# ZikangXiong/mobrob

Measured on AMD Instinct MI355X. Metric: env-steps/sec (whole node), doggo PPO, higher is better.
Workload: dtype f32

## Files before the change

### mobrob_amd/csrc/engine.hip

```cpp
#include <hip/hip_runtime.h>
#include <rccl/rccl.h>
#include <dlfcn.h>

#include <algorithm>
#include <atomic>
#include <thread>
#include <cmath>
#include <cstdarg>
#include <cstdio>
#include <climits>
#include <cstring>
#include <ctime>
#include <cstdlib>
#include <string>
#include <vector>

#ifdef MOBROB_POISON_LDS
namespace mobrob {
__global__ __launch_bounds__(1024) void k_poison_lds() {
  extern __shared__ unsigned poison_words[];
  volatile unsigned* w = poison_words;
  for (int i = threadIdx.x; i < 160 * 256; i += 1024) w[i] = 0xFFFFFFFFu;
}
inline void poison_lds(hipStream_t st) {
// ... 88 lines not shown
  int HL = 0, GL = 0;
  int tPW[kMaxHidden] = {0}, tPB[kMaxHidden] = {0}, tVW[kMaxHidden] = {0}, tVB[kMaxHidden] = {0}, tAW = 0, tAB = 0, tVWh = 0, tVBh = 0;
  int ntens = 13;
  int Bl;
  int nmb;
  int rows_max;
  int offs[kMaxTensors + 1];
  hipStream_t stream = nullptr;
  bool own_stream = false;
  float *params = nullptr, *grads = nullptr , *m = nullptr, *v = nullptr;
  NormChunk* chunks_dev = nullptr;
  double* chunk_partial = nullptr;
  int nchunks = 0;
  float *pW1p = nullptr, *vW1p = nullptr, *aWp = nullptr, *vWp = nullptr;
  int64_t adam_step = 0;
  float *obs = nullptr, *actions = nullptr, *rewards = nullptr, *es = nullptr, *values = nullptr, *logp = nullptr,
        *adv = nullptr, *ret = nullptr;
  float *last_values = nullptr, *last_dones = nullptr, *prev_dones = nullptr, *dones_tmp = nullptr;
  float *clip_act = nullptr, *rew_tmp = nullptr, *term_obs = nullptr, *term_val = nullptr, *eps_dev = nullptr;
  uint8_t *trunc_dev = nullptr, *dones_u8 = nullptr;
  int *ep_len = nullptr, *ep_len2 = nullptr;
  uint32_t* ctr_dev = nullptr;
  hipGraph_t ro_graph = nullptr;
  hipGraphExec_t ro_exec = nullptr;
  struct RolloutSpec {
    int kind = 0;
    float p_term = 0.f;
    int time_limit = 0;
    GoalEnvParams goal{};
  } ro_spec;
  int env_started = 0;
  hipStream_t vstream = nullptr;
  std::vector<hipEvent_t> ev_chunks;
  hipEvent_t ev_vdone = nullptr;
  float* gstate[2] = {nullptr, nullptr};
  double* ep_stats = nullptr;
  uint64_t ep_ring_read = 0;
  uint32_t draw_counter = 0;
  int nparts = 0;
  int part_act_t[MOBROB_MAX_PARTS] = {0}, part_store_t[MOBROB_MAX_PARTS] = {0};
  int part_obs_t[MOBROB_MAX_PARTS] = {0};
  hipEvent_t ev_part[MOBROB_MAX_PARTS] = {nullptr};
  const void* pinned_seen[8] = {nullptr};
  unsigned pinned_seen_n = 0;
  uint32_t draw_ro0 = 0;
  unsigned* srv_flags = nullptr;
  int srv_blocks = 0;
  int* srv_abort = nullptr;
  uint32_t env_step_counter = 0;
  int t = 0;
  bool rollout_ready = false;
  bool train_rec_valid = false;
  bool train_rec_external = false;
  int* rows = nullptr;
  int64_t* perm_dev = nullptr;
  double* advstat = nullptr;
  double* expvar_part = nullptr;
  unsigned long long* advbins = nullptr;
  uint64_t perm_counter = 0;
  unsigned adv_pass = 0;
  bool epoch_open = false;
  float* stats = nullptr;
  int stats_cap = 0, stats_n = 0;
  int cur_count = 0;
  bool grad_pending = false;
  double clip_vf = -1.0;
  double target_kl = -1.0;
  int last_epochs_started = 0, last_stopped_early = 0, last_steps_applied = 0;
  ncclComm_t comm = nullptr;
  int64_t allreduce_calls = 0, allreduce_bytes = 0;
  struct OneShot {
    char* xbuf = nullptr;
    size_t payload = 0;
    char* peer[kOneShotMaxRanks] = {nullptr};
    int world = 0, rank = -1;
    bool ready = false;
    unsigned long long seq = 0;
    int* error = nullptr;
    long long timeout_ticks = 0;
  } oneshot;
  double* norm_rec_sum = nullptr; int* norm_rec_t = nullptr; int* fold_idx_dev = nullptr;
  int fold_start[kMaxTensors + 1] = {0};
  bool use_norm_records = false;
  bool epoch_kernel_on = true;
  unsigned* epoch_bar = nullptr;
  float* epoch_consts = nullptr;
  int* epoch_idx = nullptr;
  char* epoch_stage = nullptr;
  int* epoch_err_host = nullptr;
  hipEvent_t epoch_ev = nullptr;
  int last_update_mode = 0;
  float* epoch_snap = nullptr;
  int rollout64_tile_max = 256;
  int pair64_min_tiles = 65;
  int split64_max_tiles = 64;
  float *Xg = nullptr, *actg = nullptr, *lpg = nullptr, *advg = nullptr, *retg = nullptr, *oldvg = nullptr;
  float *hp[kMaxHidden] = {nullptr}, *hv[kMaxHidden] = {nullptr}, *mu = nullptr, *vout = nullptr;
  float *dmu = nullptr, *dv = nullptr, *dzp[kMaxHidden] = {nullptr}, *dzv[kMaxHidden] = {nullptr};
  float *pred_obs = nullptr, *pred_act = nullptr;
  int gemm_tiles = 0;
  bool sde = false, sde_hold = false;
  float *sde_E = nullptr, *sde_E1 = nullptr, *sde_lat2 = nullptr, *sde_gsig = nullptr, *sde_graw = nullptr;
  float *sde_S2 = nullptr, *sde_var = nullptr;
  SdeMode sde_mode{1, 0};
  hipStream_t cstream = nullptr;
  hipEvent_t ev_in = nullptr, ev_k = nullptr, ev_store = nullptr;
  struct Stage {
    float *obs = nullptr, *eps = nullptr, *rew = nullptr, *term = nullptr;
    uint8_t *dones = nullptr, *trunc = nullptr;
  } stage[2];
  float *o_raw = nullptr, *o_clip = nullptr, *o_val = nullptr, *o_lp = nullptr;
  int stage_i = 0;
  bool prof_on = false;
  uint32_t prof_mask = ~0u;
  std::vector<ProfSpan> spans;
  std::vector<hipEvent_t> ev_pool;
  double prof_ms[MOBROB_K_COUNT] = {0};
  int64_t prof_calls[MOBROB_K_COUNT] = {0};
  std::vector<void*> allocs;
  char* arena = nullptr;
  size_t arena_bytes = 0, arena_used = 0;
  bool plan_only = false;
  std::vector<NormChunk> chunk_table;
  FusedState fused;
  char* eval_buf = nullptr;
  size_t eval_bytes = 0;
};

namespace {

int check_async_error(mobrob_ppo_engine* e);

constexpr size_t kArenaAlign = 256;

template <typename Tp>
int dalloc(mobrob_ppo_engine* e, Tp** p, size_t count) {
  const size_t bytes = (std::max<size_t>(count, 1) * sizeof(Tp) + kArenaAlign - 1) / kArenaAlign * kArenaAlign;
  if (e->plan_only) {
    e->arena_used += bytes;
    *p = nullptr;
    return MOBROB_OK;
  }
  if (e->arena_used + bytes > e->arena_bytes)
    return fail(MOBROB_ERR_INVALID, "device arena too small: need more than %zu bytes", e->arena_bytes);
  void* q = e->arena + e->arena_used;
  e->arena_used += bytes;
  HIPC(hipMemsetAsync(q, 0, bytes, e->stream));
  *p = static_cast<Tp*>(q);
  return MOBROB_OK;
}

hipEvent_t get_event(mobrob_ppo_engine* e) {
  if (!e->ev_pool.empty()) {
    hipEvent_t ev = e->ev_pool.back();
    e->ev_pool.pop_back();
    return ev;
  }
  hipEvent_t ev;
  (void)hipEventCreate(&ev);
  return ev;
}

struct ProfScope {
  mobrob_ppo_engine* e;
  ProfSpan s;
  bool on;
// ... 69 lines not shown
}
int gemm_tile_class(const mobrob_ppo_engine* e, const GemmOp& a) {
  const int f = e->gemm_tiles, M = a.g.M, N = a.g.N;
  if (f == 22 && M > 32 && N > 32) return 22;
  if ((f == 21 || f == 22) && M > 32) return 21;
  const long w21 = (long)cdiv(M, 64) * cdiv(N, 32) * a.ksplit, w22 = (long)cdiv(M, 64) * cdiv(N, 64) * a.ksplit;
  if (f != 0 || M <= 32 || w21 < 2048) return 11;
  return (N <= 32 || w22 < 2048) ? 21 : 22;
}
void launch_multi(mobrob_ppo_engine* e, const GemmOp* const* ops, int n) {
  GemmMulti m{};
  int gx = 1, gy = 1, z = 0;
  for (int p = 0; p < 4; ++p) {
    const GemmOp& o = *ops[p < n ? p : n - 1];
    m.g[p] = o.g; m.mode[p] = o.mode; m.epi[p] = o.epi;
    m.zbeg[p] = z;
    if (p < n) {
      z += o.ksplit;
      gx = std::max(gx, cdiv(cdiv(o.g.M, 32), 4)); gy = std::max(gy, cdiv(o.g.N, 32));
    }
  }
  m.zbeg[4] = z;
  hipLaunchKernelGGL(k_gemm_multi, dim3(gx, gy, z), dim3(256), 0, e->stream, m);
}
void run_queues(mobrob_ppo_engine* e, const GemmQueue& qa, const GemmQueue& qb, int width) {
  static const int pairing = env_int("MOBROB_GEMM_PAIR", 2);
  const size_t n = std::max(qa.size(), qb.size());
  for (size_t j0 = 0; j0 < n; j0 += width) {
    const GemmOp* st[4];
    int ns = 0;
    bool small = pairing >= 2;
    for (size_t j = j0; j < j0 + width && j < n; ++j)
      for (const GemmQueue* q : {&qa, &qb})
        if (j < q->size()) {
          st[ns++] = &(*q)[j];
          small = small && gemm_tile_class(e, (*q)[j]) == 11;
        }
    if (small && ns >= 2) { launch_multi(e, st, ns); continue; }
    for (size_t j = j0; j < j0 + width && j < n; ++j) {
      const GemmOp* a = j < qa.size() ? &qa[j] : nullptr;
      const GemmOp* b = j < qb.size() ? &qb[j] : nullptr;
      if (a && b && pairing >= 1 && a->mode == b->mode && a->epi == b->epi) { launch_op(e, *a, b); continue; }
      if (a) launch_op(e, *a);
      if (b) launch_op(e, *b);
    }
  }
}

void linear_fwd(mobrob_ppo_engine* e, const float* X, int ldx, const float* W, int ldw, const float* bias, float* Y,
                int ldy, int M, int Nn, int K, bool tanh_, float* Z = nullptr, GemmQueue* q = nullptr) {
  GemmOp o;
  GemmArgs& g = o.g;
  g.A = X; g.B = W; g.C = Y; g.M = M; g.N = Nn; g.K = K; g.lda = ldx; g.ldb = ldw; g.ldc = ldy; g.bias = bias;
  g.act = e->cfg.activation;
  g.Z = (tanh_ && act_needs_z(g.act)) ? Z : nullptr; g.ldz = ldy;
  o.mode = MODE_NT; o.epi = tanh_ ? EPI_BIAS_TANH : EPI_BIAS;
  if (q) q->push_back(o); else launch_op(e, o);
}
void linear_bwd_input(mobrob_ppo_engine* e, const float* dY, int ldd, const float* W, int ldw, const float* H, int ldh,
                      float* dZ, int ldz, float* bias_grad, int M, int Nn, int K, GemmQueue* q = nullptr) {
  GemmOp o;
  GemmArgs& g = o.g;
  g.A = dY; g.B = W; g.C = dZ; g.M = M; g.N = Nn; g.K = K; g.lda = ldd; g.ldb = ldw; g.ldc = ldz;
  g.Hact = H; g.ldh = ldh; g.colsum = bias_grad; g.act = e->cfg.activation;
  o.mode = MODE_NN; o.epi = EPI_DTANH_COLSUM;
  if (q) q->push_back(o); else launch_op(e, o);
}
void linear_bwd_weight(mobrob_ppo_engine* e, const float* dY, int ldd, const float* X, int ldx, float* dW, int ldw,
                       int M, int Nn, int rows, GemmQueue* q = nullptr) {
  GemmOp o;
  GemmArgs& g = o.g;
  g.A = dY; g.B = X; g.C = dW; g.M = M; g.N = Nn; g.K = rows; g.lda = ldd; g.ldb = ldx; g.ldc = ldw;
  const int wtiles = cdiv(M, M <= 32 ? 32 : 64) * cdiv(Nn, (M <= 32 || Nn <= 32) ? 32 : 64);
  int ksplit = std::max(1, std::min(cdiv(rows, 64), cdiv(2048, wtiles)));
  g.kchunk = rup(cdiv(rows, ksplit), 8);
  o.ksplit = cdiv(rows, g.kchunk);
  o.mode = MODE_TN; o.epi = EPI_ATOMIC;
  if (q) q->push_back(o); else launch_op(e, o);
}

float* Pp(mobrob_ppo_engine* e, int t) { return e->params + e->offs[t]; }
float* Gp(mobrob_ppo_engine* e, int t) { return e->grads + e->offs[t]; }

void pack_x3_all(mobrob_ppo_engine* e) {
  if (e->fused.net[0].W2x == nullptr) return;
  PackX3Args a{};
  const int w1[2] = {T_PW1, T_VW1}, w2[2] = {T_PW2, T_VW2};
  int maxthreads = 0;
  for (int n = 0; n < 2; ++n) {
    const int i1 = 3 * n, i2 = 3 * n + 1, i3 = 3 * n + 2;
    a.W[i1] = Pp(e, w1[n]); a.N[i1] = FH; a.K[i1] = e->D; a.ld[i1] = e->D; a.NB[i1] = FH / 32; a.KS[i1] = e->Dp / 16; a.scale[i1] = kTanhScale;
    a.out[i1] = reinterpret_cast<unsigned short*>(const_cast<unsigned*>(e->fused.net[n].W1x));
    a.W[i2] = Pp(e, w2[n]); a.N[i2] = FH; a.K[i2] = FH; a.ld[i2] = FH; a.NB[i2] = FH / 32; a.KS[i2] = FH / 16; a.scale[i2] = kTanhScale;
    a.out[i2] = reinterpret_cast<unsigned short*>(const_cast<unsigned*>(e->fused.net[n].W2x));
    a.W[i3] = Pp(e, w2[n]); a.N[i3] = FH; a.K[i3] = FH; a.ld[i3] = FH; a.NB[i3] = FH / 32; a.KS[i3] = FH / 16; a.scale[i3] = 1.0f; a.trans[i3] = 1;
    a.out[i3] = reinterpret_cast<unsigned short*>(const_cast<unsigned*>(e->fused.net[n].W2bx));
    maxthreads = std::max(maxthreads, std::max(a.NB[i1] * a.KS[i1], a.NB[i2] * a.KS[i2]) * 512);
  }
  hipLaunchKernelGGL(k_pack_x3_multi, dim3(cdiv(maxthreads, 256), 6), dim3(256), 0, e->stream, a);
  if (e->fused.train_chain) {
    ChainPackArgs c{};
    const int w3[2] = {T_AW, T_VW};
    for (int n = 0; n < 2; ++n) {
      c.W1[n] = Pp(e, w1[n]); c.W2[n] = Pp(e, w2[n]); c.W3[n] = Pp(e, w3[n]);
      c.w1c[n] = reinterpret_cast<unsigned short*>(const_cast<unsigned*>(e->fused.net[n].W1c));
      c.w2c[n] = reinterpret_cast<unsigned short*>(const_cast<unsigned*>(e->fused.net[n].W2c));
      c.w2bc[n] = reinterpret_cast<unsigned short*>(const_cast<unsigned*>(e->fused.net[n].W2bc));
      c.w3c[n] = const_cast<float*>(e->fused.net[n].W3c); c.w3bc[n] = const_cast<float*>(e->fused.net[n].W3bc);
      c.head[n] = n == 0 ? e->A : 1;
    }
    c.D = e->D; c.Dp = e->Dp;
    hipLaunchKernelGGL(k_pack_chain, dim3(FH * FH / 256, 2), dim3(256), 0, e->stream, c);
  }
}

void repack(mobrob_ppo_engine* e) {
  auto pad = [&](const float* src, float* dst, int r, int c, int rp, int cp) {
    hipLaunchKernelGGL(k_pad_rows, dim3(cdiv(rp * cp, 256)), dim3(256), 0, e->stream, src, dst, r, c, rp, cp);
  };
  pad(Pp(e, T_PW1), e->pW1p, e->H1, e->D, e->H1, e->Dp);
  pad(Pp(e, T_VW1), e->vW1p, e->G1, e->D, e->G1, e->Dp);
  pad(Pp(e, T_AW), e->aWp, e->A, e->HL, e->Ap, e->HL);
  pad(Pp(e, T_VW), e->vWp, 1, e->GL, 8, e->GL);
  fused_repack(e->fused, e->params, e->offs, e->stream);
  pack_x3_all(e);
}

void forward_generic(mobrob_ppo_engine* e, const float* X, int rows, bool want_pi, float* mu_out, bool want_v,
                     float* v_out, bool keep_z = false) {
  GemmQueue qp, qv;
  if (want_pi) {
    linear_fwd(e, X, e->Dp, e->pW1p, e->Dp, Pp(e, e->tPB[0]), e->hp[0], e->Hp[0], rows, e->Hp[0], e->Dp, true, keep_z ? e->dzp[0] : nullptr, &qp);
    for (int l = 1; l < e->Lp; ++l)
      linear_fwd(e, e->hp[l - 1], e->Hp[l - 1], Pp(e, e->tPW[l]), e->Hp[l - 1], Pp(e, e->tPB[l]), e->hp[l], e->Hp[l], rows, e->Hp[l], e->Hp[l - 1], true,
                 keep_z ? e->dzp[l] : nullptr, &qp);
    linear_fwd(e, e->hp[e->Lp - 1], e->HL, e->aWp, e->HL, Pp(e, T_AB), mu_out, e->Ap, rows, e->A, e->HL, false, nullptr, &qp);
  }
  if (want_v) {
    linear_fwd(e, X, e->Dp, e->vW1p, e->Dp, Pp(e, e->tVB[0]), e->hv[0], e->Hv[0], rows, e->Hv[0], e->Dp, true, keep_z ? e->dzv[0] : nullptr, &qv);
    for (int l = 1; l < e->Lv; ++l)
      linear_fwd(e, e->hv[l - 1], e->Hv[l - 1], Pp(e, e->tVW[l]), e->Hv[l - 1], Pp(e, e->tVB[l]), e->hv[l], e->Hv[l], rows, e->Hv[l], e->Hv[l - 1], true,
                 keep_z ? e->dzv[l] : nullptr, &qv);
    linear_fwd(e, e->hv[e->Lv - 1], e->GL, e->vWp, e->GL, Pp(e, T_VB), v_out, 1, rows, 1, e->GL, false, nullptr, &qv);
  }
  run_queues(e, qp, qv, 1);
}

void forward(mobrob_ppo_engine* e, const float* X, int rows, bool want_pi, float* mu_out, bool want_v, float* v_out) {
  if (e->fused.enabled && fused_forward(e->fused, X, rows, want_pi, mu_out, e->Ap, want_v, v_out, e->stream)) return;
  forward_generic(e, X, rows, want_pi, mu_out, want_v, v_out);
}

int value_net_width_sum(const mobrob_ppo_engine* e) {
  int s = 0;
  for (int l = 0; l < e->Lv; ++l) s += e->Hv[l];
  return s;
}
ValueNetArgs value_net_args(mobrob_ppo_engine* e) {
  ValueNetArgs vn{};
  for (int l = 0; l < e->Lv; ++l) { vn.W[l] = Pp(e, e->tVW[l]); vn.b[l] = Pp(e, e->tVB[l]); vn.G[l] = e->Hv[l]; }
  vn.Wv = Pp(e, T_VW); vn.bv = Pp(e, T_VB);
  vn.L = e->Lv; vn.act = e->cfg.activation; vn.width_sum = value_net_width_sum(e);
  return vn;
}
BootNetArgs boot_args(mobrob_ppo_engine* e) { return BootNetArgs{value_net_args(e), (float)e->cfg.gamma, e->term_val}; }

void value_flagged(mobrob_ppo_engine* e, const float* obs_rows, const uint8_t* flags, float* out,
                   float* bootstrap_rewards = nullptr) {
  const size_t sm = (size_t)(e->D + value_net_width_sum(e) + 16) * sizeof(float);
  hipLaunchKernelGGL(k_value_flagged, dim3(e->N), dim3(256), sm, e->stream, obs_rows, e->Dp, flags, value_net_args(e), e->D, out,
                     bootstrap_rewards, (float)e->cfg.gamma);
}

uint64_t eps_seed(const mobrob_ppo_engine* e) { return e->cfg.seed ^ (0xD1B54A32D192ED03ull * (uint64_t)(e->cfg.rank + 1)); }

void run_gae(mobrob_ppo_engine* e) {
  ProfScope ps(e, MOBROB_K_GAE);
  const double gl = e->cfg.gamma * e->cfg.gae_lambda;
  hipLaunchKernelGGL(k_gae, dim3(cdiv(e->N, kGaeEnvs)), dim3(kGaeThreads), 0, e->stream, e->rewards, e->values, e->es, e->last_values,
                     e->last_dones, (float)e->cfg.gamma, gl, e->T, e->N, e->adv, e->ret);
}

void sde_resample(mobrob_ppo_engine* e, int r0, int n, uint32_t draw, const uint32_t* draw_base, bool single) {
  const int HLA = e->HL * e->A, per = cdiv(HLA, 4);
  hipLaunchKernelGGL(k_sde_resample, dim3(cdiv((n + (single ? 1 : 0)) * per, 256)), dim3(256), 0, e->stream, Pp(e, T_LOGSTD), HLA, e->A, e->sde_mode, r0, n,
                     eps_seed(e) ^ 0x5DE5DE5DE5DE5DEull, draw, draw_base, e->sde_E, single ? e->sde_E1 : (float*)nullptr);
}

void sde_variance(mobrob_ppo_engine* e, int rows, bool fresh_table, float* lat2 = nullptr) {
  if (fresh_table)
    hipLaunchKernelGGL(k_sde_std2, dim3(cdiv(e->HL * e->A, 256)), dim3(256), 0, e->stream, Pp(e, T_LOGSTD), e->HL, e->A, e->sde_mode, e->sde_S2);
  hipLaunchKernelGGL(k_sde_var, dim3(cdiv(rows, 4)), dim3(256), 0, e->stream, e->hp[e->Lp - 1], e->HL, e->sde_S2, rows, e->HL, e->A, e->sde_var, e->Ap,
                     lat2);
}

void act_rows(mobrob_ppo_engine* e, int t, int r0, int n, const float* eps_dev_or_null, uint32_t draw,
              const uint32_t* draw_base, float* clip_out = nullptr) {
  ProfScope ps(e, MOBROB_K_ACT);
  if (!clip_out) clip_out = e->clip_act + (size_t)r0 * e->A;
  const size_t row = (size_t)t * e->N + r0;
  const float* X = e->obs + row * e->Dp;
  if (e->fused.enabled) {
    FusedActArgs a{};
    a.X = X; a.rows = n; a.row0 = r0; a.want_pi = 1; a.want_v = 1; a.mu = nullptr; a.ldmu = e->Ap;
    a.v = e->values + row; a.sample = 1; a.A = e->A; a.log_std = Pp(e, T_LOGSTD); a.eps = eps_dev_or_null;
    a.seed = eps_seed(e); a.draw = draw; a.draw_base = draw_base; a.lo = (float)e->cfg.action_low; a.hi = (float)e->cfg.action_high;
    a.act_raw = e->actions + row * e->A; a.act_clip = clip_out; a.logp = e->logp + row;
    fused_launch_act(e->fused, a, e->stream);
// ... 648 lines not shown
    }
    (void)hipHostFree(e->o_raw); (void)hipHostFree(e->o_clip); (void)hipHostFree(e->o_val); (void)hipHostFree(e->o_lp);
    (void)hipEventDestroy(e->ev_in); (void)hipEventDestroy(e->ev_k); (void)hipEventDestroy(e->ev_store);
    (void)hipStreamDestroy(e->cstream);
  }
  for (hipEvent_t ev : e->ev_part)
    if (ev) (void)hipEventDestroy(ev);
  if (e->srv_flags) (void)hipHostFree(e->srv_flags);
  if (e->srv_abort) (void)hipFree(e->srv_abort);
  if (e->epoch_stage) (void)hipHostFree(e->epoch_stage);
  if (e->epoch_err_host) (void)hipHostFree(e->epoch_err_host);
  if (e->epoch_ev) (void)hipEventDestroy(e->epoch_ev);
  if (e->ro_exec) (void)hipGraphExecDestroy(e->ro_exec);
  if (e->ro_graph) (void)hipGraphDestroy(e->ro_graph);
  if (e->vstream) {
    (void)hipStreamSynchronize(e->vstream);
    for (auto ev : e->ev_chunks) (void)hipEventDestroy(ev);
    (void)hipEventDestroy(e->ev_vdone);
    (void)hipStreamDestroy(e->vstream);
  }
  for (auto ev : e->ev_pool) (void)hipEventDestroy(ev);
  for (void* p : e->allocs) (void)hipFree(p);
  if (e->eval_buf) (void)hipFree(e->eval_buf);
  if (e->own_stream && e->stream) (void)hipStreamDestroy(e->stream);
  delete e;
}

int mobrob_ppo_set_stream(mobrob_ppo_engine_t* e, void* s) {
  if (!e) return fail(MOBROB_ERR_INVALID, "null engine");
  HIPC(hipStreamSynchronize(e->stream));
  if (e->ro_exec) { (void)hipGraphExecDestroy(e->ro_exec); e->ro_exec = nullptr; }
  if (e->ro_graph) { (void)hipGraphDestroy(e->ro_graph); e->ro_graph = nullptr; }
  if (e->own_stream && e->stream) HIPC(hipStreamDestroy(e->stream));
  if (s == nullptr) {
    HIPC(hipStreamCreateWithFlags(&e->stream, hipStreamNonBlocking));
    e->own_stream = true;
  } else {
    e->stream = static_cast<hipStream_t>(s);
    e->own_stream = false;
  }
  return MOBROB_OK;
}

int mobrob_ppo_synchronize(mobrob_ppo_engine_t* e) {
  if (!e) return fail(MOBROB_ERR_INVALID, "null engine");
  HIPC(hipStreamSynchronize(e->stream));
  return check_async_error(e);
}

int64_t mobrob_ppo_param_count(const mobrob_ppo_engine_t* e) { return e ? e->P : -1; }

int mobrob_ppo_get_params(mobrob_ppo_engine_t* e, float* out, int64_t n) {
  if (!e || !out || n != e->P) return fail(MOBROB_ERR_INVALID, "get_params: n=%lld, expected %d", (long long)n, e ? e->P : -1);
  HIPC(hipMemcpyAsync(out, e->params, (size_t)n * 4, hipMemcpyDeviceToHost, e->stream));
  HIPC(hipStreamSynchronize(e->stream));
  return MOBROB_OK;
}
int mobrob_ppo_set_params(mobrob_ppo_engine_t* e, const float* in, int64_t n) {
  if (!e || !in || n != e->P) return fail(MOBROB_ERR_INVALID, "set_params: n=%lld, expected %d", (long long)n, e ? e->P : -1);
  HIPC(hipMemcpyAsync(e->params, in, (size_t)n * 4, hipMemcpyHostToDevice, e->stream));
  repack(e);
  HIPC(hipStreamSynchronize(e->stream));
  return MOBROB_OK;
}
int mobrob_ppo_get_optimizer_state(mobrob_ppo_engine_t* e, float* m, float* v, int64_t n, int64_t* step) {
  if (!e || n != e->P) return fail(MOBROB_ERR_INVALID, "get_optimizer_state: bad size");
  if (m) HIPC(hipMemcpyAsync(m, e->m, (size_t)n * 4, hipMemcpyDeviceToHost, e->stream));
  if (v) HIPC(hipMemcpyAsync(v, e->v, (size_t)n * 4, hipMemcpyDeviceToHost, e->stream));
  HIPC(hipStreamSynchronize(e->stream));
  if (step) *step = e->adam_step;
  return MOBROB_OK;
}
int mobrob_ppo_set_optimizer_state(mobrob_ppo_engine_t* e, const float* m, const float* v, int64_t n, int64_t step) {
  if (!e || !m || !v || n != e->P || step < 0) return fail(MOBROB_ERR_INVALID, "set_optimizer_state: bad argument");
  HIPC(hipMemcpyAsync(e->m, m, (size_t)n * 4, hipMemcpyHostToDevice, e->stream));
  HIPC(hipMemcpyAsync(e->v, v, (size_t)n * 4, hipMemcpyHostToDevice, e->stream));
  HIPC(hipStreamSynchronize(e->stream));
  e->adam_step = step;
  return MOBROB_OK;
}

int mobrob_ppo_rollout_begin(mobrob_ppo_engine_t* e) {
  if (!e) return fail(MOBROB_ERR_INVALID, "null engine");
  e->t = 0;
  e->rollout_ready = false; e->train_rec_valid = false;
  e->nparts = 0;
  for (auto& q : e->pinned_seen) q = nullptr;
  e->pinned_seen_n = 0;
  e->draw_ro0 = e->draw_counter;
  for (int p = 0; p < MOBROB_MAX_PARTS; ++p) {
    e->part_act_t[p] = e->part_store_t[p] = 0;
    e->part_obs_t[p] = -1;
  }
  return MOBROB_OK;
}

int mobrob_ppo_act(mobrob_ppo_engine_t* e, const float* obs, const float* eps, float* a_raw, float* a_clip,
                   float* values, float* logp) {
  if (!e || !obs) return fail(MOBROB_ERR_INVALID, "act: null argument");
  if (e->t >= e->T) return fail(MOBROB_ERR_STATE, "act: rollout buffer full (t=%d, n_steps=%d)", e->t, e->T);
  CHK(streamer_init(e));
  const size_t N = e->N, A = e->A, D = e->D;
  if (!eps && is_pinned(obs) && (!a_raw || is_pinned(a_raw)) && (!a_clip || is_pinned(a_clip)) &&
      (!values || is_pinned(values)) && (!logp || is_pinned(logp))) {
    hipLaunchKernelGGL(k_pull_rows, dim3(cdiv((int)(N * e->Dp), 256)), dim3(256), 0, e->stream, obs,
                       e->obs + (size_t)e->t * N * e->Dp, (int)N, (int)D, e->Dp);
    act_slot(e, e->t, nullptr);
    auto push = [&](const float* dev, float* host, size_t n) {
      if (host) hipLaunchKernelGGL(k_copy_f32, dim3(cdiv((int)n, 256)), dim3(256), 0, e->stream, dev, host, (int)n);
    };
    push(e->clip_act, a_clip, N * A);
    push(e->actions + (size_t)e->t * N * A, a_raw, N * A);
    push(e->values + (size_t)e->t * N, values, N);
    push(e->logp + (size_t)e->t * N, logp, N);
    HIPC(hipGetLastError());
    HIPC(hipStreamSynchronize(e->stream));
    return MOBROB_OK;
  }
  auto& st = e->stage[e->stage_i];
  const float* src = stage_in(obs, st.obs, N * D);
  CHK(upload_obs_on(e, e->cstream, src, e->obs + (size_t)e->t * N * e->Dp, e->N));
  if (eps) {
    const float* es = stage_in(eps, st.eps, N * A);
    HIPC(hipMemcpyAsync(e->eps_dev, es, N * A * 4, hipMemcpyHostToDevice, e->cstream));
  }
  HIPC(hipEventRecord(e->ev_in, e->cstream));
  HIPC(hipStreamWaitEvent(e->stream, e->ev_in, 0));
  act_slot(e, e->t, eps ? e->eps_dev : nullptr);
  HIPC(hipEventRecord(e->ev_k, e->stream));
  HIPC(hipStreamWaitEvent(e->cstream, e->ev_k, 0));
  struct Out { float* user; float* stagebuf; const float* dev; size_t n; };
  const Out outs[4] = {{a_clip, e->o_clip, e->clip_act, N * A},
                       {a_raw, e->o_raw, e->actions + (size_t)e->t * N * A, N * A},
                       {values, e->o_val, e->values + (size_t)e->t * N, N},
                       {logp, e->o_lp, e->logp + (size_t)e->t * N, N}};
  bool staged[4] = {false, false, false, false};
  for (int i = 0; i < 4; ++i) {
    if (!outs[i].user) continue;
    staged[i] = !is_pinned(outs[i].user);
    HIPC(hipMemcpyAsync(staged[i] ? outs[i].stagebuf : outs[i].user, outs[i].dev, outs[i].n * 4, hipMemcpyDeviceToHost,
                        e->cstream));
  }
  HIPC(hipStreamSynchronize(e->cstream));
  for (int i = 0; i < 4; ++i)
    if (outs[i].user && staged[i]) memcpy(outs[i].user, outs[i].stagebuf, outs[i].n * 4);
  return MOBROB_OK;
}

namespace {
bool any_truncated(const uint8_t* truncated, const float* terminal_obs, int r0, int n) {
  bool any = false;
  if (truncated && terminal_obs)
    for (int i = r0; i < r0 + n; ++i) any |= truncated[i] != 0;
  return any;
}
void store_step(mobrob_ppo_engine* e, const float* rew, const uint8_t* dones, bool any_trunc) {
  const size_t o = (size_t)e->t * e->N;
  if (any_trunc) value_flagged(e, e->term_obs, e->trunc_dev, e->term_val);
  hipLaunchKernelGGL(k_store_step, dim3(cdiv(e->N, 256)), dim3(256), 0, e->stream, rew, e->prev_dones,
                     any_trunc ? e->trunc_dev : nullptr, e->term_val, (float)e->cfg.gamma, e->N, e->rewards + o, e->es + o);
  hipLaunchKernelGGL(k_u8_to_f32, dim3(cdiv(e->N, 256)), dim3(256), 0, e->stream, dones, e->prev_dones, e->N);
}
}

int mobrob_ppo_store(mobrob_ppo_engine_t* e, const float* rewards, const uint8_t* dones, const uint8_t* truncated,
                     const float* terminal_obs) {
  if (!e || !rewards || !dones) return fail(MOBROB_ERR_INVALID, "store: null argument");
  if (e->t >= e->T) return fail(MOBROB_ERR_STATE, "store: rollout buffer full");
  CHK(streamer_init(e));
  const size_t N = e->N, D = e->D;
  const bool any_trunc = any_truncated(truncated, terminal_obs, 0, e->N);
  if (is_pinned(rewards) && is_pinned(dones) && (!truncated || is_pinned(truncated)) &&
      (!terminal_obs || is_pinned(terminal_obs))) {
    if (any_trunc) {
      hipLaunchKernelGGL(k_pull_rows, dim3(cdiv((int)(N * e->Dp), 256)), dim3(256), 0, e->stream, terminal_obs, e->term_obs,
                         (int)N, (int)D, e->Dp);
      HIPC(hipMemcpyAsync(e->trunc_dev, truncated, N, hipMemcpyHostToDevice, e->stream));
    }
    store_step(e, rewards, dones, any_trunc);
    HIPC(hipGetLastError());
    e->t++;
    return MOBROB_OK;
  }
  auto& st = e->stage[e->stage_i];
  memcpy(st.rew, rewards, N * 4);
  memcpy(st.dones, dones, N);
  HIPC(hipMemcpyAsync(e->rew_tmp, st.rew, N * 4, hipMemcpyHostToDevice, e->cstream));
  HIPC(hipMemcpyAsync(e->dones_u8, st.dones, N, hipMemcpyHostToDevice, e->cstream));
  if (any_trunc) {
    memcpy(st.trunc, truncated, N);
    memcpy(st.term, terminal_obs, N * D * 4);
    HIPC(hipMemcpyAsync(e->trunc_dev, st.trunc, N, hipMemcpyHostToDevice, e->cstream));
    CHK(upload_obs_on(e, e->cstream, st.term, e->term_obs, e->N));
  }
  HIPC(hipEventRecord(e->ev_store, e->cstream));
  HIPC(hipStreamWaitEvent(e->stream, e->ev_store, 0));
  store_step(e, e->rew_tmp, e->dones_u8, any_trunc);
  HIPC(hipEventRecord(e->ev_k, e->stream));
  HIPC(hipStreamWaitEvent(e->cstream, e->ev_k, 0));
  HIPC(hipGetLastError());
  e->stage_i ^= 1;
  e->t++;
  return MOBROB_OK;
}

namespace {
int part_range(mobrob_ppo_engine* e, int part, int nparts, int* r0, int* n) {
  if (nparts < 1 || nparts > MOBROB_MAX_PARTS || nparts > e->N || part < 0 || part >= nparts)
    return fail(MOBROB_ERR_INVALID, "part %d of %d (1..%d parts, at most one per env)", part, nparts, MOBROB_MAX_PARTS);
  if (e->nparts == 0) e->nparts = nparts;
  if (e->nparts != nparts) return fail(MOBROB_ERR_STATE, "nparts changed from %d to %d inside a rollout", e->nparts, nparts);
  *r0 = (int)((int64_t)e->N * part / nparts);
  *n = (int)((int64_t)e->N * (part + 1) / nparts) - *r0;
  return MOBROB_OK;
}
}

int mobrob_ppo_act_part(mobrob_ppo_engine_t* e, int32_t part, int32_t nparts, const float* obs, float* a_clip) {
  if (!e || !obs || !a_clip) return fail(MOBROB_ERR_INVALID, "act_part: null argument");
  int r0, n;
  CHK(part_range(e, part, nparts, &r0, &n));
  const int t = e->part_act_t[part];
  if (t >= e->T) return fail(MOBROB_ERR_STATE, "act_part: rollout buffer full (part %d, t=%d)", part, t);
  if (t != e->part_store_t[part]) return fail(MOBROB_ERR_STATE, "act_part: part %d acted on step %d but has not stored it", part, t - 1);
  if (!is_pinned_cached(e, obs) || !is_pinned_cached(e, a_clip))
    return fail(MOBROB_ERR_INVALID, "act_part needs device-visible pinned buffers (mobrob_ppo_host_alloc)");
  if (!e->ev_part[part]) HIPC(hipEventCreateWithFlags(&e->ev_part[part], hipEventDisableTiming));
  const size_t D = e->D, A = e->A;
  if (e->part_obs_t[part] != t)
    hipLaunchKernelGGL(k_pull_rows, dim3(cdiv(n * e->Dp, 256)), dim3(256), 0, e->stream, obs + (size_t)r0 * D,
                       e->obs + ((size_t)t * e->N + r0) * e->Dp, n, (int)D, e->Dp);
  act_rows(e, t, r0, n, nullptr, e->draw_ro0 + (uint32_t)t, nullptr, a_clip + (size_t)r0 * A);
  HIPC(hipGetLastError());
  HIPC(hipEventRecord(e->ev_part[part], e->stream));
  e->part_act_t[part] = t + 1;
  if (e->draw_counter < e->draw_ro0 + (uint32_t)t + 1) e->draw_counter = e->draw_ro0 + (uint32_t)t + 1;
  return MOBROB_OK;
}

int mobrob_ppo_wait_part(mobrob_ppo_engine_t* e, int32_t part) {
  if (!e || part < 0 || part >= MOBROB_MAX_PARTS || !e->ev_part[part])
    return fail(MOBROB_ERR_STATE, "wait_part: part %d has no act_part in flight", part);
  HIPC(hipEventSynchronize(e->ev_part[part]));
  return MOBROB_OK;
}

int mobrob_ppo_store_part(mobrob_ppo_engine_t* e, int32_t part, int32_t nparts, const float* rewards,
                          const uint8_t* dones, const uint8_t* truncated, const float* terminal_obs,
                          const float* next_obs) {
  if (!e || !rewards || !dones) return fail(MOBROB_ERR_INVALID, "store_part: null argument");
  int r0, n;
  CHK(part_range(e, part, nparts, &r0, &n));
  const int t = e->part_store_t[part];
  if (t + 1 != e->part_act_t[part]) return fail(MOBROB_ERR_STATE, "store_part: part %d has no acted step to store (t=%d)", part, t);
  if (!is_pinned_cached(e, rewards) || !is_pinned_cached(e, dones) || (truncated && !is_pinned_cached(e, truncated)) ||
      (terminal_obs && !is_pinned_cached(e, terminal_obs)) || (next_obs && !is_pinned_cached(e, next_obs)))
    return fail(MOBROB_ERR_INVALID, "store_part needs device-visible pinned buffers (mobrob_ppo_host_alloc)");
  const bool any = any_truncated(truncated, terminal_obs, r0, n);
  const size_t o = (size_t)t * e->N + r0;
  StorePullArgs a{};
  a.rew_in = rewards + r0; a.dones = dones + r0;
  a.trunc = any ? truncated + r0 : nullptr; a.term_obs = any ? terminal_obs + (size_t)r0 * e->D : nullptr;
  a.vn = value_net_args(e);
  a.D = e->D; a.Dp = e->Dp; a.n = n; a.gamma = (float)e->cfg.gamma;
  a.prev_dones = e->prev_dones + r0; a.rew_out = e->rewards + o; a.es_out = e->es + o; a.term_val = e->term_val + r0;
  if (next_obs) {
    a.next_obs = next_obs + (size_t)r0 * e->D;
    a.obs_slot = e->obs + ((size_t)(t + 1) * e->N + r0) * e->Dp;
    e->part_obs_t[part] = t + 1;
  }
  const size_t sm = (size_t)(e->D + value_net_width_sum(e) + 32) * sizeof(float);
  hipLaunchKernelGGL(k_store_pull_part, dim3(cdiv(n, kPartRows)), dim3(256), sm, e->stream, a);
  HIPC(hipGetLastError());
  e->part_store_t[part] = t + 1;
  int tmin = e->T;
  for (int p = 0; p < nparts; ++p) tmin = std::min(tmin, e->part_store_t[p]);
  e->t = tmin;
  return MOBROB_OK;
}

int mobrob_ppo_finish_rollout(mobrob_ppo_engine_t* e, const float* last_obs, const uint8_t* dones) {
  if (!e || !last_obs || !dones) return fail(MOBROB_ERR_INVALID, "finish_rollout: null argument");
  if (e->t != e->T) return fail(MOBROB_ERR_STATE, "finish_rollout: %d of %d steps stored", e->t, e->T);
  CHK(streamer_init(e));
  const size_t N = e->N;
  auto& st = e->stage[e->stage_i];
  float* slot = e->obs + (size_t)e->T * N * e->Dp;
  const float* src = stage_in(last_obs, st.obs, N * e->D);
  CHK(upload_obs_on(e, e->cstream, src, slot, e->N));
  memcpy(st.dones, dones, N);
  HIPC(hipMemcpyAsync(e->dones_u8, st.dones, N, hipMemcpyHostToDevice, e->cstream));
  HIPC(hipEventRecord(e->ev_in, e->cstream));
  HIPC(hipStreamWaitEvent(e->stream, e->ev_in, 0));
  hipLaunchKernelGGL(k_u8_to_f32, dim3(cdiv(e->N, 256)), dim3(256), 0, e->stream, e->dones_u8, e->last_dones, e->N);
  forward(e, slot, e->N, false, nullptr, true, e->last_values);
  run_gae(e);
  HIPC(hipStreamSynchronize(e->stream));
  e->rollout_ready = true; e->train_rec_valid = false;
  return MOBROB_OK;
}

int mobrob_ppo_compute_gae(mobrob_ppo_engine_t* e) {
  if (!e) return fail(MOBROB_ERR_INVALID, "null engine");
  run_gae(e);
  HIPC(hipStreamSynchronize(e->stream));
  e->rollout_ready = true; e->train_rec_valid = false;
  return MOBROB_OK;
}

int mobrob_ppo_x3_mode(const mobrob_ppo_engine_t* e) {
  if (!e || !e->fused.enabled || e->fused.net[0].W2x == nullptr) return 0;
  return 1 | (e->fused.train_x3 ? 2 : 0) | (e->fused.train_x3 && e->fused.train_chain ? 4 : 0);
}

int mobrob_ppo_update_mode(const mobrob_ppo_engine_t* e) { return e ? e->last_update_mode : 0; }

int mobrob_ppo_explained_variance(mobrob_ppo_engine_t* e, double* out) {
  if (!e || !out) return fail(MOBROB_ERR_INVALID, "explained_variance: null argument");
  if (!e->rollout_ready) return fail(MOBROB_ERR_STATE, "explained_variance: rollout not finished");
  const int n = e->N * e->T;
  hipLaunchKernelGGL(k_explained_variance_partials, dim3(kEvBlocks), dim3(256), 0, e->stream, e->values, e->ret, n, e->expvar_part);
  double part[kEvBlocks * 4];
  HIPC(hipMemcpyAsync(part, e->expvar_part, sizeof part, hipMemcpyDeviceToHost, e->stream));
  HIPC(hipStreamSynchronize(e->stream));
  double s[4] = {0.0, 0.0, 0.0, 0.0};
  for (int b = 0; b < kEvBlocks; ++b)
    for (int k = 0; k < 4; ++k) s[k] += part[b * 4 + k];
  const double var_y = s[1] / n - (s[0] / n) * (s[0] / n), var_d = s[3] / n - (s[2] / n) * (s[2] / n);
  *out = var_y > 0.0 ? 1.0 - var_d / var_y : NAN;
  return MOBROB_OK;
}

int mobrob_ppo_mark_rollout_ready(mobrob_ppo_engine_t* e) {
  if (!e) return fail(MOBROB_ERR_INVALID, "null engine");
  e->rollout_ready = true; e->train_rec_valid = false;
  e->t = e->T;
  return MOBROB_OK;
}

namespace {
uint64_t env_seed_of(const mobrob_ppo_engine* e) {
  return e->cfg.seed ^ (0x9E3779B97F4A7C15ull * (uint64_t)(e->cfg.rank + 1));
}

bool rollout_persistent_ok(const mobrob_ppo_engine* e) {
  return e->cfg.rollout_persistent && e->fused.enabled;
}
int rollout_side_stream_init(mobrob_ppo_engine* e) {
  if (!e->vstream) {
    HIPC(hipStreamCreateWithFlags(&e->vstream, hipStreamNonBlocking));
    HIPC(hipEventCreateWithFlags(&e->ev_vdone, hipEventDisableTiming));
  }
  while ((int)e->ev_chunks.size() < e->T / 16 + 2) {
    hipEvent_t ev;
    HIPC(hipEventCreateWithFlags(&ev, hipEventDisableTiming));
    e->ev_chunks.push_back(ev);
  }
  return MOBROB_OK;
}

RolloutArgs rollout_args(mobrob_ppo_engine* e) {
  RolloutArgs a{};
  a.pi = e->fused.net[0];
  a.log_std = Pp(e, T_LOGSTD); a.seed = eps_seed(e);
  a.lo = (float)e->cfg.action_low; a.hi = (float)e->cfg.action_high;
// ... 68 lines not shown
    a.t0 = t0; a.t1 = std::min(T, t0 + pl.chunk);
    launch_rollout_kernel(e, a);
    if (pl.overlap && a.t1 < T) {
      hipEvent_t ev = e->ev_chunks[t0 / pl.chunk];
      HIPC(hipEventRecord(ev, e->stream));
      HIPC(hipStreamWaitEvent(e->vstream, ev, 0));
      value_rows(e, e->vstream, t0 * N, a.t1 * N, pl.vgrid_max);
    }
  }
  return MOBROB_OK;
}
int value_rollout_tail(mobrob_ppo_engine* e, const ChunkPlan& pl, int rows_end) {
  ProfScope ps(e, MOBROB_K_ACT);
  const int done_rows = pl.overlap ? ((e->T - 1) / pl.chunk) * pl.chunk * e->N : 0;
  value_rows(e, e->stream, done_rows, rows_end, 256);
  if (pl.overlap && done_rows > 0) {
    HIPC(hipEventRecord(e->ev_vdone, e->vstream));
    HIPC(hipStreamWaitEvent(e->stream, e->ev_vdone, 0));
  }
  return MOBROB_OK;
}

int end_device_steps(mobrob_ppo_engine* e) {
  hipLaunchKernelGGL(k_add_counters, dim3(1), dim3(64), 0, e->stream, e->ctr_dev, (uint32_t)e->T, (uint32_t)e->T);
  HIPC(hipMemcpyAsync(e->last_dones, e->prev_dones, (size_t)e->N * 4, hipMemcpyDeviceToDevice, e->stream));
  return MOBROB_OK;
}

int enqueue_rollout_persistent(mobrob_ppo_engine* e, const mobrob_ppo_engine::RolloutSpec& sp) {
  const int N = e->N, T = e->T;
  const size_t slot = (size_t)N * e->Dp;
  HIPC(hipMemcpyAsync(e->obs, e->obs + (size_t)T * slot, slot * 4, hipMemcpyDeviceToDevice, e->stream));
  if (wide_nets(e) && !e->fused.train_x3) pack_x3_all(e);
  RolloutArgs a = rollout_args(e);
  a.kind = sp.kind; a.env_seed = env_seed_of(e); a.draw_base = e->ctr_dev; a.step_base = e->ctr_dev + 1;
  a.p_term = sp.p_term; a.time_limit = sp.time_limit; a.goal = sp.goal;
  const ChunkPlan pl = chunk_plan(wide_nets(e), cdiv(N, 32), rollout64_tile_kernel(e), T, N);
  CHK(enqueue_rollout_chunks(e, a, pl));
  CHK(end_device_steps(e));
  CHK(value_rollout_tail(e, pl, (T + 1) * N));
  run_gae(e);
  return MOBROB_OK;
}

int enqueue_rollout(mobrob_ppo_engine* e, const mobrob_ppo_engine::RolloutSpec& sp) {
  if (rollout_persistent_ok(e)) return enqueue_rollout_persistent(e, sp);
  const int N = e->N, Dp = e->Dp, per = Dp / 4;
  const size_t slot = (size_t)N * Dp;
  const uint64_t env_seed = env_seed_of(e);
  HIPC(hipMemcpyAsync(e->obs, e->obs + (size_t)e->T * slot, slot * 4, hipMemcpyDeviceToDevice, e->stream));
  const BootNetArgs bt = boot_args(e);
  const size_t sm = env_step_lds_bytes(Dp, value_net_width_sum(e));
  for (int t = 0; t < e->T; ++t) {
    act_slot(e, t, nullptr, true);
    {
      ProfScope ps(e, MOBROB_K_ENV);
      if (sp.kind == 1) {
        hipLaunchKernelGGL(k_env_step_store, dim3(cdiv(N * per, 256)), dim3(256), sm, e->stream, env_seed, (uint32_t)t,
                           e->ctr_dev + 1, N, e->D, Dp, sp.p_term, sp.time_limit, e->ep_len, e->ep_len2,
                           e->obs + (size_t)(t + 1) * slot, e->term_obs, e->prev_dones, e->dones_tmp, e->trunc_dev,
                           e->rewards + (size_t)t * N, e->es + (size_t)t * N, bt);
        std::swap(e->ep_len, e->ep_len2);
      } else {
        GoalEnvArgs g{};
        g.seed = env_seed; g.step_rel = (uint32_t)t; g.step_base = e->ctr_dev + 1;
        g.N = N; g.D = e->D; g.Dp = Dp; g.A = e->A; g.p = sp.goal;
        g.act = e->clip_act; g.st_in = e->gstate[0]; g.st_out = e->gstate[1];
        g.obs_next = e->obs + (size_t)(t + 1) * slot; g.term_obs = e->term_obs;
        g.prev_dones = e->prev_dones; g.next_dones = e->dones_tmp; g.trunc = e->trunc_dev;
        g.rew_out = e->rewards + (size_t)t * N; g.es_out = e->es + (size_t)t * N; g.ep_stats = e->ep_stats;
        hipLaunchKernelGGL(k_goal_env_step_store, dim3(cdiv(N * per, 256)), dim3(256), sm, e->stream, g, bt);
        std::swap(e->gstate[0], e->gstate[1]);
      }
    }
    std::swap(e->prev_dones, e->dones_tmp);
  }
  CHK(end_device_steps(e));
  forward(e, e->obs + (size_t)e->T * slot, N, false, nullptr, true, e->last_values);
  run_gae(e);
  return MOBROB_OK;
}

int collect_device(mobrob_ppo_engine* e, const mobrob_ppo_engine::RolloutSpec& sp) {
  const int N = e->N, Dp = e->Dp, per = Dp / 4;
  const size_t slot = (size_t)N * Dp;
  if (e->env_started != sp.kind) {
    float* last = e->obs + (size_t)e->T * slot;
    if (sp.kind == 1) {
      hipLaunchKernelGGL(k_env_reset, dim3(cdiv(N * per, 256)), dim3(256), 0, e->stream, env_seed_of(e), N, e->D, Dp, last,
                         e->ep_len);
    } else {
      hipLaunchKernelGGL(k_goal_env_reset, dim3(cdiv(N * per, 256)), dim3(256), 0, e->stream, env_seed_of(e), N, e->D, Dp,
                         sp.goal, e->gstate[0], last);
      HIPC(hipMemsetAsync(e->ep_stats, 0, kEpStatsDoubles * sizeof(double), e->stream));
      e->ep_ring_read = 0;
    }
    std::vector<float> ones(N, 1.0f);
    HIPC(hipMemcpyAsync(e->prev_dones, ones.data(), (size_t)N * 4, hipMemcpyHostToDevice, e->stream));
    HIPC(hipStreamSynchronize(e->stream));
    e->env_started = sp.kind;
  }
  e->rollout_ready = false; e->train_rec_valid = false;
  if (rollout_persistent_ok(e)) CHK(rollout_side_stream_init(e));
  bool use_graph = e->cfg.rollout_graph && e->T % 2 == 0 && !rollout_persistent_ok(e);
  if (use_graph && (e->ro_exec == nullptr || memcmp(&e->ro_spec, &sp, sizeof sp) != 0)) {
    HIPC(hipStreamSynchronize(e->stream));
    if (e->ro_exec) { (void)hipGraphExecDestroy(e->ro_exec); e->ro_exec = nullptr; }
    if (e->ro_graph) { (void)hipGraphDestroy(e->ro_graph); e->ro_graph = nullptr; }
    const bool prof = e->prof_on;
    e->prof_on = false;
    hipError_t be = hipStreamBeginCapture(e->stream, hipStreamCaptureModeThreadLocal);
    if (be != hipSuccess) {
      (void)hipGetLastError();
      e->prof_on = prof;
      e->cfg.rollout_graph = 0;
      use_graph = false;
    } else {
      const int rc = enqueue_rollout(e, sp);
      hipError_t ce = hipStreamEndCapture(e->stream, &e->ro_graph);
      e->prof_on = prof;
      if (rc != MOBROB_OK) return rc;
      if (ce != hipSuccess) return fail(MOBROB_ERR_HIP, "hipStreamEndCapture: %s", hipGetErrorString(ce));
      HIPC(hipGraphInstantiate(&e->ro_exec, e->ro_graph, nullptr, nullptr, 0));
      memcpy(&e->ro_spec, &sp, sizeof sp);
    }
  }
  if (!use_graph) {
    CHK(enqueue_rollout(e, sp));
  } else {
    ProfScope ps(e, MOBROB_K_ACT);
    HIPC(hipGraphLaunch(e->ro_exec, e->stream));
  }
  HIPC(hipGetLastError());
  e->t = e->T;
  e->rollout_ready = true; e->train_rec_valid = false;
  return MOBROB_OK;
}

int collect_host_served(mobrob_ppo_engine* e, mobrob_env_step_range_fn step_range, void* env, int nparts, float* obs,
                        float* actions_clipped, float* rewards, uint8_t* dones, uint8_t* truncated, float* terminal_obs, bool* served) {
  *served = false;
  const int mode = env_int("MOBROB_COLLECT_SERVER", 1);
  const int N = e->N, T = e->T, Dp = e->Dp;
  const int rblocks = cdiv(N, 32);
  if (mode == 0) return MOBROB_OK;
  const char* why = nullptr;
  int cus = 0;
  const bool wide = e->fused.enabled && wide_nets(e);
  if (!rollout_persistent_ok(e)) why = "the fused persistent rollout kernels are off for this engine";
  else if (wide && !rollout_s8(e)) why = "not a 256-wide x3 engine with the eight-wave rollout kernel";
  else if (!wide && (e->fused.H != GH || !rollout64_tile_kernel(e))) why = "not a 64-wide engine within the tile kernel's range";
  else if (getenv("MOBROB_COLLECT_TIMING") || env_int("MOBROB_COLLECT_THREADS", 0) != 0) why = "an instrumented / threaded collector was asked for";
  else if (nparts < 1 || nparts > MOBROB_MAX_PARTS || (nparts > 1 && (N % nparts != 0 || (N / nparts) % 32 != 0))) why = "row ranges are not whole 32-row tiles";
  else if (hipDeviceGetAttribute(&cus, hipDeviceAttributeMultiprocessorCount, e->cfg.device_id) != hipSuccess || rblocks > cus) why = "more tiles than compute units";
  else if (env_int("MOBROB_DP_SAME_DEVICE", 0) != 0 && e->cfg.world_size > 1) why = "several data-parallel ranks share this device (MOBROB_DP_SAME_DEVICE)";
  else if (getenv("HSA_CU_MASK") || getenv("ROC_GLOBAL_CU_MASK")) why = "a compute-unit mask is set (HSA_CU_MASK / ROC_GLOBAL_CU_MASK)";
  else {
    const size_t N_ = (size_t)N;
    const struct { const void* p; size_t bytes; } bufs[6] = {{obs, N_ * e->D * 4}, {actions_clipped, N_ * e->A * 4}, {rewards, N_ * 4},
                                                              {dones, N_}, {truncated, N_}, {terminal_obs, N_ * e->D * 4}};
    for (const auto& b : bufs)
      if (!why) why = served_buffer_problem(b.p, b.bytes);
  }
  constexpr int kLeaseDevices = 64;
  static std::atomic<int> cus_serving[kLeaseDevices];
  std::atomic<int>& dev_lease = cus_serving[(unsigned)e->cfg.device_id % kLeaseDevices];
// ... 331 lines not shown
int mobrob_ctrl_turtlebot3(mobrob_ppo_engine_t* e, int32_t n, int32_t dev_ptrs, const float* pos, const float* theta,
                           const float* goal, const float* gain_changes, float* twist) {
  if (!e || n < 1 || !pos || !theta || !goal || !gain_changes || !twist)
    return fail(MOBROB_ERR_INVALID, "ctrl_turtlebot3: bad argument");
  CtrlBuf b{e, dev_ptrs != 0, {}, {}};
  const float *dp, *dt, *dg, *da;
  float* dtw;
  CHK(b.in(pos, (size_t)2 * n, &dp)); CHK(b.in(theta, (size_t)n, &dt)); CHK(b.in(goal, (size_t)2 * n, &dg));
  CHK(b.in(gain_changes, (size_t)2 * n, &da)); CHK(b.inout(twist, (size_t)2 * n, &dtw, false));
  hipLaunchKernelGGL(k_ctrl_turtlebot3, dim3(cdiv(n, 256)), dim3(256), 0, e->stream, n, dp, dt, dg, da, dtw);
  HIPC(hipGetLastError());
  return b.finish();
}

int mobrob_ctrl_drone_pid(mobrob_ppo_engine_t* e, int32_t n, int32_t dev_ptrs, const mobrob_drone_params_t* prm,
                          const float* pos, const float* rpy, const float* goal, const float* action, float* ctrl_state,
                          float* out) {
  if (!e || n < 1 || !prm || !pos || !rpy || !goal || !action || !ctrl_state || !out)
    return fail(MOBROB_ERR_INVALID, "ctrl_drone_pid: bad argument");
  if (!(prm->dt > 0.f) || !(prm->mass > 0.f)) return fail(MOBROB_ERR_INVALID, "ctrl_drone_pid: dt and mass must be positive");
  CtrlBuf b{e, dev_ptrs != 0, {}, {}};
  const float *dp, *dr, *dg, *da;
  float *ds, *dout;
  CHK(b.in(pos, (size_t)3 * n, &dp)); CHK(b.in(rpy, (size_t)3 * n, &dr)); CHK(b.in(goal, (size_t)3 * n, &dg));
  CHK(b.in(action, (size_t)18 * n, &da)); CHK(b.inout(ctrl_state, (size_t)12 * n, &ds, true));
  CHK(b.inout(out, (size_t)4 * n, &dout, false));
  DroneCtrlParams p{prm->mass, prm->g, prm->dt, prm->max_thrust, prm->max_xy_torque, prm->max_z_torque, prm->max_roll_pitch,
                    prm->tune_fac};
  hipLaunchKernelGGL(k_ctrl_drone_pid, dim3(cdiv(n, 256)), dim3(256), 0, e->stream, n, p, dp, dr, dg, da, ds, dout);
  HIPC(hipGetLastError());
  return b.finish();
}

int mobrob_ppo_num_minibatches(const mobrob_ppo_engine_t* e) { return e ? e->nmb : -1; }

int mobrob_ppo_epoch_begin(mobrob_ppo_engine_t* e, const int64_t* perm) {
  if (!e) return fail(MOBROB_ERR_INVALID, "null engine");
  if (!e->rollout_ready) return fail(MOBROB_ERR_STATE, "epoch_begin: rollout not finished (finish_rollout / collect first)");
  const int total = e->N * e->T;
  if (perm) {
    std::vector<uint64_t> seen(((size_t)total + 63) / 64, 0);
    for (int i = 0; i < total; ++i) {
      const int64_t v = perm[i];
      if (v < 0 || v >= total) return fail(MOBROB_ERR_INVALID, "epoch_begin: perm[%d] = %lld is outside [0, %d)", i, (long long)v, total);
      uint64_t& w = seen[(size_t)v >> 6];
      const uint64_t bit = 1ull << (v & 63);
      if (w & bit) return fail(MOBROB_ERR_INVALID, "epoch_begin: perm holds index %lld twice (not a permutation of [0, %d))", (long long)v, total);
      w |= bit;
    }
  }
  ensure_train_records(e);
  AdvStatArgs as{};
  as.adv = e->adv; as.total = total; as.T = e->T; as.N = e->N; as.bl = e->Bl; as.nmb = e->nmb;
  as.bins = e->advbins;
  unsigned* maxw = reinterpret_cast<unsigned*>(e->advbins + (size_t)2 * e->nmb);
  as.absmax_bits = maxw + (e->adv_pass & 1); as.absmax_next = maxw + ((e->adv_pass + 1) & 1);
  e->adv_pass++;
  if (perm) {
    HIPC(hipMemcpyAsync(e->perm_dev, perm, (size_t)total * 8, hipMemcpyHostToDevice, e->stream));
    hipLaunchKernelGGL(k_perm_from_host, dim3(cdiv(total, 256)), dim3(256), 0, e->stream, e->perm_dev, total, e->T,
                       e->N, e->Bl, e->rows);
    as.mb_of_row = reinterpret_cast<const int*>(e->perm_dev);
  } else {
    const uint64_t key = (e->cfg.seed * 0x9E3779B97F4A7C15ull) ^ ((uint64_t)(e->cfg.rank + 1) << 48) ^ (e->perm_counter + 1);
    e->perm_counter++;
    as.half_bits = feistel_half_bits((uint64_t)total); as.k0 = (uint32_t)key; as.k1 = (uint32_t)(key >> 32);
    hipLaunchKernelGGL(k_perm_feistel, dim3(cdiv(total, 256)), dim3(256), 0, e->stream, total, e->T, e->N,
                       as.half_bits, as.k0, as.k1, e->rows, (int64_t*)nullptr);
  }
  const int sgrid = std::max(1, std::min(256, cdiv(total, 4 * 1024)));
  const size_t slds = e->nmb <= kAdvLdsMinibatches ? (size_t)2 * e->nmb * adv_bin_replicas(e->nmb) * sizeof(unsigned long long) : 0;
  hipLaunchKernelGGL(k_adv_absmax, dim3(sgrid), dim3(1024), 0, e->stream, as);
  hipLaunchKernelGGL(k_adv_stats_stream, dim3(sgrid), dim3(1024), slds, e->stream, as);
  hipLaunchKernelGGL(k_adv_fold, dim3(cdiv(e->nmb, 64)), dim3(64), 0, e->stream, as, e->advstat);
  HIPC(hipGetLastError());
  e->epoch_open = true;
  return MOBROB_OK;
}

int mobrob_ppo_minibatch_grad(mobrob_ppo_engine_t* e, int32_t mb) {
  if (!e) return fail(MOBROB_ERR_INVALID, "null engine");
  if (!e->epoch_open) return fail(MOBROB_ERR_STATE, "minibatch_grad before epoch_begin");
  if (mb < 0 || mb >= e->nmb) return fail(MOBROB_ERR_INVALID, "minibatch %d out of range [0,%d)", mb, e->nmb);
  const int start = mb * e->Bl, B = std::min(e->Bl, e->N * e->T - start);
  const float inv_bg = 1.0f / (float)((int64_t)B * e->cfg.world_size);
  e->cur_count = B;
  if (!e->fused.enabled) generic_minibatch_grad(e, mb, start, B, inv_bg);
  else if (e->fused.H == 64) fused64_minibatch_grad(e, mb, start, B, inv_bg);
  else fused_minibatch_grad(e, mb, start, B, inv_bg);
  HIPC(hipGetLastError());
  e->grad_pending = true;
  return MOBROB_OK;
}

namespace {
void fill_adam_pack_args(mobrob_ppo_engine* e, AdamPackArgs& a) {
  a.p = e->params; a.g = e->grads; a.m = e->m; a.v = e->v; a.P = e->P;
  a.chunks = e->chunks_dev; a.partial = e->chunk_partial; a.nchunks = e->nchunks;
  if (e->use_norm_records) {
    a.partial = e->norm_rec_sum; a.fold_idx = e->fold_idx_dev;
    for (int i = 0; i <= kMaxTensors; ++i) a.fold_start[i] = e->fold_start[i];
  }
  a.max_norm = (float)e->cfg.max_grad_norm; a.beta1 = (float)e->cfg.adam_beta1; a.beta2 = (float)e->cfg.adam_beta2;
  a.eps = (float)e->cfg.adam_eps;
  for (int i = 0; i <= kMaxTensors; ++i) a.offs[i] = e->offs[i];
  a.ntens = e->ntens; a.two_by_two = e->Lp == 2 && e->Lv == 2; a.id_pw1 = T_PW1; a.id_vw1 = T_VW1; a.id_aw = T_AW; a.id_vw = T_VW; a.HL = e->HL; a.GL = e->GL;
  a.D = e->D; a.Dp = e->Dp; a.A = e->A; a.Ap = e->Ap; a.H1 = e->H1; a.H2 = e->H2; a.G1 = e->G1; a.G2 = e->G2;
  a.pW1p = e->pW1p; a.vW1p = e->vW1p; a.aWp = e->aWp; a.vWp = e->vWp;
  for (int n = 0; n < 2; ++n) {
    const bool on = e->fused.enabled;
    a.fW1f[n] = on ? (float*)e->fused.net[n].W1f : nullptr;
    a.fW2f[n] = on ? (float*)e->fused.net[n].W2f : nullptr;
    a.fW3f[n] = on ? (float*)e->fused.net[n].W3f : nullptr;
    const bool ch = on && e->fused.train_chain;
    a.fW2b[n] = on && !ch ? (float*)e->fused.net[n].W2b : nullptr;
    a.fW3b[n] = on && !ch ? (float*)e->fused.net[n].W3b : nullptr;
    a.fW3h[n] = (on && (n == 1 || e->fused.A <= 16)) ? (float*)e->fused.net[n].W3h : nullptr;
    a.fb1s[n] = on ? (float*)e->fused.net[n].b1s : nullptr;
    a.fb2s[n] = on ? (float*)e->fused.net[n].b2s : nullptr;
    const bool x3 = on && e->fused.train_x3;
    a.xW1[n] = x3 ? reinterpret_cast<unsigned short*>(const_cast<unsigned*>(e->fused.net[n].W1x)) : nullptr;
    a.xW2[n] = x3 ? reinterpret_cast<unsigned short*>(const_cast<unsigned*>(e->fused.net[n].W2x)) : nullptr;
    a.xW2b[n] = x3 && !ch ? reinterpret_cast<unsigned short*>(const_cast<unsigned*>(e->fused.net[n].W2bx)) : nullptr;
    a.cW1[n] = ch ? reinterpret_cast<unsigned short*>(const_cast<unsigned*>(e->fused.net[n].W1c)) : nullptr;
    a.cW2[n] = ch ? reinterpret_cast<unsigned short*>(const_cast<unsigned*>(e->fused.net[n].W2c)) : nullptr;
    a.cW2b[n] = ch ? reinterpret_cast<unsigned short*>(const_cast<unsigned*>(e->fused.net[n].W2bc)) : nullptr;
    a.cW3[n] = ch ? const_cast<float*>(e->fused.net[n].W3c) : nullptr;
    a.cW3b[n] = ch ? const_cast<float*>(e->fused.net[n].W3bc) : nullptr;
  }
}
}

namespace {
struct AdamStep { float step_size, bc2_sqrt; };
AdamStep next_adam_step(mobrob_ppo_engine* e) {
  e->adam_step++;
  const double bc1 = 1.0 - std::pow(e->cfg.adam_beta1, (double)e->adam_step), bc2 = 1.0 - std::pow(e->cfg.adam_beta2, (double)e->adam_step);
  return {(float)(e->cfg.learning_rate / bc1), (float)std::sqrt(bc2)};
}
int next_stats_row(mobrob_ppo_engine* e) {
  if (e->stats_n >= e->stats_cap) e->stats_n = 0;
  return e->stats_n++;
}
StatsArgs apply_norms(mobrob_ppo_engine* e) {
  StatsArgs st = stats_args(e);
  st.stats_row = e->stats + (size_t)next_stats_row(e) * 8;
  st.inv_bg = 1.0f / (float)((int64_t)e->cur_count * e->cfg.world_size);
  if (!e->use_norm_records)
    hipLaunchKernelGGL(k_sqnorm_chunks, dim3(e->nchunks), dim3(256), 0, e->stream, e->grads, e->chunks_dev,
                       e->chunk_partial, st);
  return st;
}
int apply_adam(mobrob_ppo_engine* e, const StatsArgs& st) {
  const AdamStep step = next_adam_step(e);
  AdamPackArgs a{};
  fill_adam_pack_args(e, a);
  a.step_size = step.step_size; a.bc2_sqrt = step.bc2_sqrt;
  if (e->use_norm_records) a.st = st;
  a.stats_row = st.stats_row;
  a.loss_sums_zero = e->fused.enabled ? e->grads + e->P : nullptr;
  hipLaunchKernelGGL(k_adam_pack, dim3(cdiv(e->P, 256)), dim3(256), 0, e->stream, a);
  HIPC(hipGetLastError());
  e->grad_pending = false;
  return MOBROB_OK;
}
}

namespace {
int apply_checked(mobrob_ppo_engine* e, int32_t* stopped) {
  *stopped = 0;
  ProfScope ps(e, MOBROB_K_APPLY);
  const StatsArgs st = apply_norms(e);
  if (e->target_kl > 0.0) {
    float approx_kl = 0.f;
    HIPC(hipMemcpyAsync(&approx_kl, st.stats_row + 4, sizeof(float), hipMemcpyDeviceToHost, e->stream));
    HIPC(hipStreamSynchronize(e->stream));
    if ((double)approx_kl > 1.5 * e->target_kl) {
      *stopped = 1;
      e->grad_pending = false;
      HIPC(hipMemsetAsync(st.stats_row + 6, 0xFF, sizeof(float), e->stream));
      if (e->fused.enabled) HIPC(hipMemsetAsync(e->grads + e->P, 0, 8 * sizeof(float), e->stream));
      return MOBROB_OK;
    }
  }
  return apply_adam(e, st);
}
}

int mobrob_ppo_minibatch_apply(mobrob_ppo_engine_t* e) {
  if (!e) return fail(MOBROB_ERR_INVALID, "null engine");
  if (!e->grad_pending) return fail(MOBROB_ERR_STATE, "minibatch_apply without a pending gradient");
  if (e->target_kl > 0.0)
    return fail(MOBROB_ERR_STATE, "target_kl is set: a step-wise driver must call mobrob_ppo_minibatch_apply_checked and honour its stop flag");
  int32_t stopped = 0;
  return apply_checked(e, &stopped);
}

int mobrob_ppo_minibatch_apply_checked(mobrob_ppo_engine_t* e, int32_t* stopped) {
  if (!e || !stopped) return fail(MOBROB_ERR_INVALID, "minibatch_apply_checked: null argument");
  if (!e->grad_pending) return fail(MOBROB_ERR_STATE, "minibatch_apply without a pending gradient");
  return apply_checked(e, stopped);
}

int mobrob_ppo_sde_reset_noise(mobrob_ppo_engine_t* e) {
  if (!e) return fail(MOBROB_ERR_INVALID, "null engine");
  if (!e->sde) return fail(MOBROB_ERR_STATE, "sde_reset_noise: the engine was not created with use_sde");
  sde_resample(e, 0, e->N, e->draw_counter++, nullptr, true);
  HIPC(hipGetLastError());
  return MOBROB_OK;
}

int mobrob_ppo_sde_set_noise(mobrob_ppo_engine_t* e, const float* z) {
  if (!e) return fail(MOBROB_ERR_INVALID, "null engine");
  if (!e->sde) return fail(MOBROB_ERR_STATE, "sde_set_noise: the engine was not created with use_sde");
  if (e->sde_hold != (z != nullptr) && e->ro_exec) {
    HIPC(hipStreamSynchronize(e->stream));
    (void)hipGraphExecDestroy(e->ro_exec); e->ro_exec = nullptr;
    if (e->ro_graph) { (void)hipGraphDestroy(e->ro_graph); e->ro_graph = nullptr; }
  }
  e->sde_hold = z != nullptr;
  if (!z) return MOBROB_OK;
  const size_t HLA = (size_t)e->HL * e->A, n = (size_t)e->N * HLA;
  if (n > (size_t)1 << 30) return fail(MOBROB_ERR_INVALID, "sde_set_noise: too many matrix elements");
  HIPC(hipMemcpyAsync(e->sde_E, z, n * 4, hipMemcpyHostToDevice, e->stream));
  hipLaunchKernelGGL(k_sde_from_z, dim3(cdiv((int)n, 256)), dim3(256), 0, e->stream, e->sde_E, Pp(e, T_LOGSTD), (int)HLA, e->A, e->sde_mode, (int)n, e->sde_E);
  hipLaunchKernelGGL(k_copy_f32, dim3(cdiv((int)HLA, 256)), dim3(256), 0, e->stream, e->sde_E, e->sde_E1, (int)HLA);
  HIPC(hipGetLastError());
  HIPC(hipStreamSynchronize(e->stream));
  return MOBROB_OK;
}

int mobrob_ppo_set_hyper(mobrob_ppo_engine_t* e, int32_t which, double value) {
  if (!e) return fail(MOBROB_ERR_INVALID, "null engine");
  switch (which) {
    case MOBROB_HYPER_LEARNING_RATE:
      if (!(value >= 0.0)) return fail(MOBROB_ERR_INVALID, "learning_rate must be >= 0");
      e->cfg.learning_rate = value; break;
    case MOBROB_HYPER_CLIP_RANGE:
      if (!(value >= 0.0)) return fail(MOBROB_ERR_INVALID, "clip_range must be >= 0");
      e->cfg.clip_range = value; break;
    case MOBROB_HYPER_CLIP_RANGE_VF: e->clip_vf = value >= 0.0 ? value : -1.0; break;
    case MOBROB_HYPER_TARGET_KL: e->target_kl = value > 0.0 ? value : -1.0; break;
    case MOBROB_HYPER_ENT_COEF: e->cfg.ent_coef = value; break;
    case MOBROB_HYPER_VF_COEF: e->cfg.vf_coef = value; break;
// ... 35 lines not shown
  decltype(&ncclGetErrorString) GetErrorString = nullptr;
  decltype(&ncclCommCount) CommCount = nullptr;
  decltype(&ncclCommUserRank) CommUserRank = nullptr;
};
RcclApi g_rccl;
int rccl_load() {
  if (g_rccl.lib) return MOBROB_OK;
  void* h = dlopen("librccl.so.1", RTLD_NOW | RTLD_GLOBAL);
  if (!h) h = dlopen("librccl.so", RTLD_NOW | RTLD_GLOBAL);
  if (!h) return fail(MOBROB_ERR_STATE, "RCCL not found: %s", dlerror());
#define RSYM(field, name)                                                     \
  g_rccl.field = reinterpret_cast<decltype(g_rccl.field)>(dlsym(h, name));   \
  if (!g_rccl.field) return fail(MOBROB_ERR_STATE, "RCCL symbol %s missing", name);
  RSYM(GetUniqueId, "ncclGetUniqueId")
  RSYM(CommInitRank, "ncclCommInitRank")
  RSYM(CommDestroy, "ncclCommDestroy")
  RSYM(AllReduce, "ncclAllReduce")
  RSYM(GetErrorString, "ncclGetErrorString")
  RSYM(CommCount, "ncclCommCount")
  RSYM(CommUserRank, "ncclCommUserRank")
#undef RSYM
  g_rccl.lib = h;
  return MOBROB_OK;
}
#define NCCLC(expr)                                                                                   \
  do {                                                                                                \
    ncclResult_t _r = (expr);                                                                         \
    if (_r != ncclSuccess) return fail(MOBROB_ERR_HIP, "%s failed: %s", #expr, g_rccl.GetErrorString(_r)); \
  } while (0)

size_t oneshot_payload_bytes(const mobrob_ppo_engine* e) {
  const size_t need = std::max((size_t)(e->P + 8) * sizeof(float), (size_t)e->nmb * 4 * sizeof(double));
  return (need + 255) / 256 * 256;
}
int oneshot_all_reduce(mobrob_ppo_engine* e, void* buf, size_t count, int dtype) {
  auto& o = e->oneshot;
  const size_t bytes = count * (dtype == 1 ? sizeof(double) : sizeof(float));
  if (bytes > o.payload) return fail(MOBROB_ERR_INVALID, "one-shot all-reduce: message of %zu bytes, exchange slot of %zu", bytes, o.payload);
  o.seq++;
  OneShotArgs a{};
  const size_t slot = (size_t)(o.seq & 1) * o.payload;
  a.local = buf; a.mine = o.xbuf + slot; a.my_flags = reinterpret_cast<unsigned long long*>(o.xbuf + 2 * o.payload);
  for (int r = 0; r < o.world; ++r) {
    a.peer[r] = o.peer[r] + slot;
    a.peer_flags[r] = reinterpret_cast<const unsigned long long*>(o.peer[r] + 2 * o.payload);
  }
  a.world = o.world; a.rank = o.rank; a.bytes = bytes; a.seq = o.seq; a.error = o.error; a.timeout_ticks = o.timeout_ticks;
  a.fence_form = env_int("MOBROB_ONESHOT_FENCE", 0) != 0;
  const int chunks = cdiv((int)bytes, kOneShotChunkBytes);
  if (dtype == 1) hipLaunchKernelGGL(k_oneshot_allreduce<double>, dim3(chunks), dim3(256), 0, e->stream, a);
  else hipLaunchKernelGGL(k_oneshot_allreduce<float>, dim3(chunks), dim3(256), 0, e->stream, a);
  HIPC(hipGetLastError());
  return MOBROB_OK;
}
int check_async_error(mobrob_ppo_engine* e) {
  if (e->epoch_err_host && *(volatile int*)e->epoch_err_host != 0) {
    *(volatile int*)e->epoch_err_host = 0;
    return fail(MOBROB_ERR_STATE, "the co-operative epoch kernel gave up at a grid barrier (a workgroup never arrived: another tenant on the "
                                  "device?); the update of this train() is incomplete -- MOBROB_EPOCH_KERNEL=0 runs the three launches per step");
  }
  if (e->oneshot.error && *(volatile int*)e->oneshot.error != 0) {
    const int v = *(volatile int*)e->oneshot.error;
    *(volatile int*)e->oneshot.error = 0;
    return fail(MOBROB_ERR_STATE, "one-shot all-reduce: a peer rank never published message %d (dead or stalled rank)", v - 1);
  }
  return MOBROB_OK;
}

int dp_all_reduce(mobrob_ppo_engine* e, void* buf, size_t count, int dtype, mobrob_allreduce_fn fn, void* ctx) {
  ProfScope ps(e, MOBROB_K_ALLREDUCE);
  e->allreduce_calls++;
  e->allreduce_bytes += count * (dtype == 1 ? 8 : 4);
  if (fn) {
    const int r = fn(ctx, buf, count, dtype, (void*)e->stream);
    return r == 0 ? MOBROB_OK : fail(MOBROB_ERR_STATE, "all-reduce callback returned %d", r);
  }
  if (e->oneshot.ready) return oneshot_all_reduce(e, buf, count, dtype);
  NCCLC(g_rccl.AllReduce(buf, buf, count, dtype == 1 ? ncclDouble : ncclFloat, ncclSum, e->comm, e->stream));
  return MOBROB_OK;
}
}

namespace {
bool norm_records_wanted(const mobrob_ppo_engine* e, bool dp) {
  return !dp && e->fused.enabled && e->target_kl <= 0.0 && !env_switched_off("MOBROB_NO_NORM_RECORDS");
}
struct EpochLaunch { int grid = 0, group = 0; };
bool epoch_kernel_eligible(const mobrob_ppo_engine* e, bool dp, bool records, EpochLaunch* launch) {
  static_assert(kEpochRedBlocks * 256 >= 10 * 1024 + 200 && (kEpochRedBlocks - 1) * 256 < 10 * 1024 + 200, "kEpochRedBlocks = ceil(s64_size() / 256)");
  const FusedState& f = e->fused;
  if (dp || e->cfg.world_size != 1 || !e->epoch_kernel_on || !f.enabled || f.H != GH || e->epoch_bar == nullptr) return false;
  if (e->target_kl > 0.0 || !records || kEpochRedBlocks != cdiv(s64_size(), 256)) return false;
  if (e->prof_on && (e->prof_mask & ((1u << MOBROB_K_GRAD_REDUCE) | (1u << MOBROB_K_APPLY))) != 0) return false;
  const Grad64Plan pl = grad64_plan(e, std::min(e->Bl, e->N * e->T));
  if (!pl.split) return false;
  int cus = 0;
  if (hipDeviceGetAttribute(&cus, hipDeviceAttributeMultiprocessorCount, e->cfg.device_id) != hipSuccess) return false;
  launch->grid = std::max(2 * pl.ntiles, 2 * kEpochRedBlocks); launch->group = pl.group;
  return launch->grid <= cus;
}
constexpr size_t kEpochLdsBytes = 84 * 1024;

int launch_epoch_kernel(mobrob_ppo_engine* e, int ep, const EpochLaunch& launch) {
  if (!e->use_norm_records) return fail(MOBROB_ERR_STATE, "k_epoch64 outside train_loop's norm-record scope");
  const int total = e->N * e->T, nmb = e->nmb;
  const size_t slot_bytes = (size_t)nmb * 12;
  if (!e->epoch_stage) {
    HIPC(hipHostMalloc((void**)&e->epoch_stage, slot_bytes * (size_t)std::max(1, e->cfg.n_epochs), hipHostMallocDefault));
    HIPC(hipHostMalloc((void**)&e->epoch_err_host, sizeof(int), hipHostMallocCoherent | hipHostMallocMapped));
    *e->epoch_err_host = 0;
    HIPC(hipEventCreateWithFlags(&e->epoch_ev, hipEventDisableTiming));
  }
  if (ep == 0) HIPC(hipEventSynchronize(e->epoch_ev));
  char* slot = e->epoch_stage + slot_bytes * (size_t)(ep % std::max(1, e->cfg.n_epochs));
  float* consts = reinterpret_cast<float*>(slot);
  int* idx = reinterpret_cast<int*>(slot + (size_t)nmb * 8);
  for (int mb = 0; mb < nmb; ++mb) {
    const AdamStep step = next_adam_step(e);
    consts[2 * mb] = step.step_size; consts[2 * mb + 1] = step.bc2_sqrt;
    idx[mb] = next_stats_row(e);
  }
  HIPC(hipMemcpyAsync(e->epoch_consts, consts, (size_t)nmb * 8, hipMemcpyHostToDevice, e->stream));
  HIPC(hipMemcpyAsync(e->epoch_idx, idx, (size_t)nmb * 4, hipMemcpyHostToDevice, e->stream));
  HIPC(hipEventRecord(e->epoch_ev, e->stream));
  HIPC(hipMemsetAsync(e->epoch_bar, 0, 1024 * sizeof(unsigned), e->stream));
  Epoch64Args ea{};
  ea.tr = train64_args(e);
  ea.rd = slab64_reduce_args(e);
  ea.rd.group = launch.group;
  fill_adam_pack_args(e, ea.ad);
  ea.ad.st = stats_args(e);
  ea.ad.loss_sums_zero = e->grads + e->P;
  ea.rows = e->rows; ea.advstat = e->advstat;
  ea.total = total; ea.bl = e->Bl; ea.nmb = nmb; ea.world = e->cfg.world_size;
  ea.step_consts = e->epoch_consts; ea.stats_idx = e->epoch_idx; ea.stats = e->stats;
  ea.barrier = e->epoch_bar; ea.error_host = e->epoch_err_host;
  ea.timeout_ticks = (long long)(env_double("MOBROB_EPOCH_TIMEOUT_S", 10.0) * 1e8);
  void* kargs[1] = {&ea};
  {
    ProfScope ps(e, MOBROB_K_TRAIN_GRAD);
    hipError_t le = hipSuccess;
    FUSED_DISPATCH_DP(e->Dp, FUSED64_DISPATCH_NJ(e->A, {
      const void* fn = reinterpret_cast<const void*>(k_epoch64<DPc, NJc>);
      le = hipFuncSetAttribute(fn, hipFuncAttributeMaxDynamicSharedMemorySize, (int)kEpochLdsBytes);
      if (le == hipSuccess) le = hipLaunchCooperativeKernel(fn, dim3(launch.grid), dim3(256), kargs, (unsigned)kEpochLdsBytes, e->stream);
    }));
    if (le != hipSuccess) return fail(MOBROB_ERR_HIP, "k_epoch64 launch (%d workgroups): %s", launch.grid, hipGetErrorString(le));
  }
  e->cur_count = std::min(e->Bl, total - (nmb - 1) * e->Bl);
  e->grad_pending = false;
  e->last_steps_applied += nmb;
  return MOBROB_OK;
}

int train_loop(mobrob_ppo_engine* e, const int64_t* perms, bool dp, bool records, mobrob_allreduce_fn fn, void* ctx) {
  if (!dp && e->cfg.world_size != 1)
    return fail(MOBROB_ERR_STATE, "mobrob_ppo_train is the single-rank loop; data-parallel ranks call mobrob_ppo_train_dp "
                                  "(or drive epoch_begin/minibatch_grad/[all-reduce]/minibatch_apply)");
  const size_t total = (size_t)e->N * e->T;
  e->stats_n = 0;
  const bool kl = e->target_kl > 0.0;
  e->last_epochs_started = 0; e->last_stopped_early = 0; e->last_steps_applied = 0;
  struct RecordsOn {
    mobrob_ppo_engine* e;
    RecordsOn(mobrob_ppo_engine* e_, bool on) : e(e_) { e->use_norm_records = on; }
    ~RecordsOn() { e->use_norm_records = false; }
  } records_on(e, records);
  EpochLaunch epoch_launch;
  const bool epoch_kernel = epoch_kernel_eligible(e, dp, records, &epoch_launch);
  e->last_update_mode = epoch_kernel ? 1 : 0;
  for (int ep = 0; ep < e->cfg.n_epochs; ++ep) {
    CHK(mobrob_ppo_epoch_begin(e, perms ? perms + (size_t)ep * total : nullptr));
    if (dp) CHK(dp_all_reduce(e, e->advstat, (size_t)e->nmb * 4, 1, fn, ctx));
    e->last_epochs_started = ep + 1;
    if (ep == e->cfg.n_epochs - 1 || kl) e->stats_n = 0;
    if (epoch_kernel) {
      CHK(launch_epoch_kernel(e, ep, epoch_launch));
      continue;
    }
    for (int mb = 0; mb < e->nmb && !e->last_stopped_early; ++mb) {
      CHK(mobrob_ppo_minibatch_grad(e, mb));
      if (dp) CHK(dp_all_reduce(e, e->grads, (size_t)e->P + 8, 0, fn, ctx));
      int32_t stopped = 0;
      CHK(apply_checked(e, &stopped));
      if (stopped) {
        e->last_stopped_early = 1;
        break;
      }
      e->last_steps_applied++;
    }
    if (e->last_stopped_early) break;
  }
  e->epoch_open = false;
  return MOBROB_OK;
}
int copy_optimizer_state(mobrob_ppo_engine* e, bool restore) {
  float* const live[3] = {e->params, e->m, e->v};
  for (int i = 0; i < 3; ++i) {
    float* const snap = e->epoch_snap + (size_t)i * e->P;
    HIPC(hipMemcpyAsync(restore ? live[i] : snap, restore ? snap : live[i], (size_t)e->P * sizeof(float), hipMemcpyDeviceToDevice, e->stream));
  }
  return MOBROB_OK;
}
}

extern "C" {

int mobrob_ppo_train_enqueue(mobrob_ppo_engine_t* e, const int64_t* perms) {
  if (!e) return fail(MOBROB_ERR_INVALID, "null engine");
  return train_loop(e, perms, false, norm_records_wanted(e, false), nullptr, nullptr);
}

int mobrob_ppo_comm_unique_id(uint8_t* out128) {
  if (!out128) return fail(MOBROB_ERR_INVALID, "comm_unique_id: null argument");
  static_assert(sizeof(ncclUniqueId) == 128, "ncclUniqueId is 128 bytes");
  CHK(rccl_load());
  ncclUniqueId id;
  NCCLC(g_rccl.GetUniqueId(&id));
  memcpy(out128, &id, sizeof id);
  return MOBROB_OK;
}
int mobrob_ppo_comm_prepare(mobrob_ppo_engine_t* e) {
  if (!e) return fail(MOBROB_ERR_INVALID, "comm_prepare: null engine");
  if (e->comm) return fail(MOBROB_ERR_STATE, "comm_prepare: the engine already has a communicator");
  CHK(rccl_load());
  HIPC(hipSetDevice(e->cfg.device_id));
  return MOBROB_OK;
}
int mobrob_ppo_comm_init_rank(mobrob_ppo_engine_t* e, const uint8_t* id128, int32_t rank, int32_t nranks) {
  if (!e || !id128) return fail(MOBROB_ERR_INVALID, "comm_init: null argument");
  if (nranks != e->cfg.world_size)
    return fail(MOBROB_ERR_INVALID, "comm_init: %d ranks, but the engine splits its minibatch for world_size %d", nranks, e->cfg.world_size);
  if (rank < 0 || rank >= nranks) return fail(MOBROB_ERR_INVALID, "comm_init: rank %d of %d", rank, nranks);
  CHK(mobrob_ppo_comm_prepare(e));
  ncclUniqueId id;
  memcpy(&id, id128, sizeof id);
  NCCLC(g_rccl.CommInitRank(&e->comm, nranks, id, rank));
  return MOBROB_OK;
}
int mobrob_ppo_comm_init(mobrob_ppo_engine_t* e, const uint8_t* id128) {
  if (!e) return fail(MOBROB_ERR_INVALID, "comm_init: null argument");
  return mobrob_ppo_comm_init_rank(e, id128, e->cfg.rank, e->cfg.world_size);
}
int mobrob_ppo_comm_info(mobrob_ppo_engine_t* e, int32_t* nranks, int32_t* rank) {
  if (!e) return fail(MOBROB_ERR_INVALID, "null engine");
  int n = 0, r = -1;
  if (e->comm) {
    NCCLC(g_rccl.CommCount(e->comm, &n));
    NCCLC(g_rccl.CommUserRank(e->comm, &r));
  }
// ... 127 lines not shown
  const size_t sbytes = std::max((size_t)nf * sizeof(float), (size_t)nd * sizeof(double));
  HIPC(hipMalloc((void**)&scratch, sbytes + 256));
  if (hipMalloc((void**)&bad, sizeof(int)) != hipSuccess) { (void)hipFree(scratch); return fail(MOBROB_ERR_HIP, "exchange_selfcheck: hipMalloc"); }
  (void)hipMemsetAsync(bad, 0, sizeof(int), e->stream);
  int rc = MOBROB_OK;
  for (unsigned msg = 0; msg < 4 && rc == MOBROB_OK; ++msg) {
    const int dtype = msg >> 1, n = dtype ? nd : nf;
    if (dtype) hipLaunchKernelGGL(k_selfcheck_fill<double>, dim3(cdiv(n, 256)), dim3(256), 0, e->stream, reinterpret_cast<double*>(scratch), n, rank, msg);
    else hipLaunchKernelGGL(k_selfcheck_fill<float>, dim3(cdiv(n, 256)), dim3(256), 0, e->stream, reinterpret_cast<float*>(scratch), n, rank, msg);
    if (which == 1) rc = oneshot_all_reduce(e, scratch, (size_t)n, dtype);
    else if (g_rccl.AllReduce(scratch, scratch, (size_t)n, dtype ? ncclDouble : ncclFloat, ncclSum, e->comm, e->stream) != ncclSuccess)
      rc = fail(MOBROB_ERR_HIP, "exchange_selfcheck: ncclAllReduce failed");
    if (rc != MOBROB_OK) break;
    if (dtype) hipLaunchKernelGGL(k_selfcheck_compare<double>, dim3(cdiv(n, 256)), dim3(256), 0, e->stream, reinterpret_cast<const double*>(scratch), n, world, msg, bad);
    else hipLaunchKernelGGL(k_selfcheck_compare<float>, dim3(cdiv(n, 256)), dim3(256), 0, e->stream, reinterpret_cast<const float*>(scratch), n, world, msg, bad);
  }
  if (rc == MOBROB_OK) {
    int h = -1;
    hipError_t er = hipMemcpyAsync(&h, bad, sizeof(int), hipMemcpyDeviceToHost, e->stream);
    if (er == hipSuccess) er = hipStreamSynchronize(e->stream);
    if (er != hipSuccess) rc = fail(MOBROB_ERR_HIP, "exchange_selfcheck: %s", hipGetErrorString(er));
    else *mismatches = h;
  }
  (void)hipStreamSynchronize(e->stream);
  (void)hipFree(bad);
  (void)hipFree(scratch);
  if (rc != MOBROB_OK) return rc;
  if (which == 1) CHK(check_async_error(e));
  return MOBROB_OK;
}
int mobrob_ppo_allreduce_counters(mobrob_ppo_engine_t* e, int64_t* calls, int64_t* bytes, int32_t reset) {
  if (!e) return fail(MOBROB_ERR_INVALID, "null engine");
  if (calls) *calls = e->allreduce_calls;
  if (bytes) *bytes = e->allreduce_bytes;
  if (reset) { e->allreduce_calls = 0; e->allreduce_bytes = 0; }
  return MOBROB_OK;
}

int mobrob_ppo_train(mobrob_ppo_engine_t* e, const int64_t* perms, mobrob_ppo_train_stats_t* st) {
  if (!e) return fail(MOBROB_ERR_INVALID, "null engine");
  const bool records = norm_records_wanted(e, false);
  EpochLaunch launch_unused;
  const bool snap = e->cfg.world_size == 1 && e->epoch_snap != nullptr && epoch_kernel_eligible(e, false, records, &launch_unused);
  const int64_t adam_step0 = e->adam_step; const uint64_t perm_counter0 = e->perm_counter;
  if (snap) CHK(copy_optimizer_state(e, false));
  CHK(train_loop(e, perms, false, records, nullptr, nullptr));
  if (snap && (e->last_update_mode & 1)) {
    HIPC(hipStreamSynchronize(e->stream));
    if (e->epoch_err_host && *(volatile int*)e->epoch_err_host != 0) {
      *(volatile int*)e->epoch_err_host = 0;
      fprintf(stderr, "[mobrob_ppo] the co-operative epoch kernel gave up at a grid barrier (workgroups not resident together: other spinning tenants "
                      "on the device?); the update is re-run as three launches per optimizer step and this engine keeps that form\n");
      CHK(copy_optimizer_state(e, true));
      HIPC(hipMemsetAsync(e->grads + e->P, 0, 8 * sizeof(float), e->stream));
      repack(e);
      e->adam_step = adam_step0; e->perm_counter = perm_counter0;
      e->epoch_kernel_on = false;
      CHK(train_loop(e, perms, false, records, nullptr, nullptr));
    }
  }
  if (st) {
    std::vector<float> rows((size_t)e->nmb * 8);
    const int n = mobrob_ppo_fetch_step_stats(e, rows.data(), e->nmb);
    if (n < 0) return n;
    double acc[7] = {0};
    int n_norm = 0;
    for (int i = 0; i < n; ++i) {
      for (int k = 0; k < 6; ++k) acc[k] += rows[(size_t)i * 8 + k];
      if (!std::isnan(rows[(size_t)i * 8 + 6])) { acc[6] += rows[(size_t)i * 8 + 6]; n_norm++; }
    }
    const double d = n > 0 ? n : 1;
    st->policy_loss = (float)(acc[0] / d); st->value_loss = (float)(acc[1] / d); st->entropy_loss = (float)(acc[2] / d);
    st->loss = (float)(acc[3] / d); st->approx_kl = (float)(acc[4] / d); st->clip_fraction = (float)(acc[5] / d);
    st->grad_norm = (float)(acc[6] / (n_norm > 0 ? n_norm : 1)); st->n_minibatches = e->last_steps_applied;
  } else {
    HIPC(hipStreamSynchronize(e->stream));
  }
  return MOBROB_OK;
}

int mobrob_ppo_predict(mobrob_ppo_engine_t* e, const float* obs, int32_t n, int32_t deterministic, const float* eps,
                       float* actions, float* values) {
  if (!e || !obs || n < 1) return fail(MOBROB_ERR_INVALID, "predict: bad argument");
  for (int s = 0; s < n; s += e->rows_max) {
    const int c = std::min(e->rows_max, n - s);
    CHK(upload_obs(e, obs + (size_t)s * e->D, e->pred_obs, c));
    forward(e, e->pred_obs, c, actions != nullptr, e->mu, values != nullptr, e->vout);
    if (actions) {
      float* scratch = e->pred_act;
      if (deterministic) {
        hipLaunchKernelGGL(k_clip_mean, dim3(cdiv(c * e->A, 256)), dim3(256), 0, e->stream, e->mu, e->Ap, c, e->A,
                           (float)e->cfg.action_low, (float)e->cfg.action_high, scratch);
      } else {
        if (e->sde) {
          const bool own = n == e->N;
          sde_variance(e, c, true);
          hipLaunchKernelGGL(k_sample_sde, dim3(cdiv(c, 4)), dim3(256), 0, e->stream, e->mu, e->Ap, e->hp[e->Lp - 1], e->HL, e->sde_var, e->Ap,
                             own ? e->sde_E : e->sde_E1, s, own ? 0 : 1, c, e->HL, e->A, (float)e->cfg.action_low, (float)e->cfg.action_high,
                             (float*)nullptr, scratch, (float*)nullptr);
          HIPC(hipMemcpyAsync(actions + (size_t)s * e->A, scratch, (size_t)c * e->A * 4, hipMemcpyDeviceToHost, e->stream));
          if (values) HIPC(hipMemcpyAsync(values + s, e->vout, (size_t)c * 4, hipMemcpyDeviceToHost, e->stream));
          HIPC(hipStreamSynchronize(e->stream));
          continue;
        }
        const float* epsd = nullptr;
        if (eps) {
          HIPC(hipMemcpyAsync(e->eps_dev, eps + (size_t)s * e->A, (size_t)c * e->A * 4, hipMemcpyHostToDevice, e->stream));
          epsd = e->eps_dev;
        }
        hipLaunchKernelGGL(k_sample, dim3(cdiv(c, 256)), dim3(256), 0, e->stream, e->mu, e->Ap, Pp(e, T_LOGSTD), epsd,
                           c, e->A, (float)e->cfg.action_low, (float)e->cfg.action_high, eps_seed(e), e->draw_counter,
                           (const uint32_t*)nullptr, (float*)nullptr, scratch, (float*)nullptr);
        e->draw_counter++;
      }
      HIPC(hipMemcpyAsync(actions + (size_t)s * e->A, scratch, (size_t)c * e->A * 4, hipMemcpyDeviceToHost, e->stream));
    }
    if (values) HIPC(hipMemcpyAsync(values + s, e->vout, (size_t)c * 4, hipMemcpyDeviceToHost, e->stream));
    HIPC(hipStreamSynchronize(e->stream));
  }
  return MOBROB_OK;
}

static int grow_eval_buf(mobrob_ppo_engine_t* e, size_t need) {
  if (need > e->eval_bytes) {
    HIPC(hipStreamSynchronize(e->stream));
    if (e->eval_buf) HIPC(hipFree(e->eval_buf));
    e->eval_buf = nullptr;
    e->eval_bytes = 0;
    HIPC(hipMalloc(reinterpret_cast<void**>(&e->eval_buf), need));
    e->eval_bytes = need;
  }
  return MOBROB_OK;
}

static GoalEnvParams eval_env_params(const mobrob_goal_env_t* env, int A, bool terminate_on_goal, int time_limit) {
  GoalEnvParams g{};
  g.P = env->pos_dim; g.terminate_on_goal = terminate_on_goal; g.time_limit = time_limit;
  g.dt = env->dt; g.extent = env->extent; g.reach = env->reach_radius; g.bonus = env->goal_bonus;
  g.extra_bonus = env->extra_bonus; g.noise = env->obs_noise;
  for (int j = 0; j < 3; ++j)
    for (int k = 0; k < 32; ++k) g.mix[j][k] = (j < env->pos_dim && k < A) ? env->mix[j][k] : 0.f;
  return g;
}

extern "C++" {
struct EvalCall {
  const char* who;
  int N, max_steps, deterministic;
  uint64_t seed;
  int trace_robots, trace_steps;
  float* trace_out;
  int trace_extra = 0;
  bool tracing() const { return trace_out && trace_robots > 0 && trace_steps > 0; }
  size_t trace_floats() const { return (size_t)trace_steps * trace_robots; }
};

static int eval_check_dims(const mobrob_ppo_engine_t* e, const mobrob_goal_env_t* env, const char* who) {
  if (env->pos_dim < 1 || env->pos_dim > 3 || 3 * env->pos_dim > e->D)
    return fail(MOBROB_ERR_INVALID, "%s: pos_dim must be 1..3 and 3*pos_dim <= obs_dim", who);
  if (e->A > 32) return fail(MOBROB_ERR_INVALID, "%s: act_dim must be <= 32", who);
  return MOBROB_OK;
}
static int eval_check_actions_trace(const mobrob_ppo_engine_t* e, const EvalCall& c) {
  if (!c.deterministic && e->sde)
    return fail(MOBROB_ERR_INVALID, "%s: stochastic actions of a use_sde policy are not supported (deterministic only)", c.who);
  if (c.tracing() && (c.trace_robots > c.N || c.trace_steps > c.max_steps))
    return fail(MOBROB_ERR_INVALID, "%s: trace_robots <= n_robots and trace_steps <= max_steps", c.who);
  return MOBROB_OK;
}

struct EvalCarve {
  size_t total = 0;
  size_t add(size_t bytes) {
    const size_t off = total;
    total += (bytes + 255) / 256 * 256;
    return off;
  }
};
template <class T>
static T* eval_at(const mobrob_ppo_engine_t* e, size_t off) { return reinterpret_cast<T*>(e->eval_buf + off); }

static int eval_prepare(mobrob_ppo_engine_t* e, const EvalCall& c, const GoalEnvParams& p, EvalCarve& carve, EvalArgs& a) {
  const int N = c.N, Dp = e->Dp, Ap = e->Ap;
  const bool tracing = c.tracing();
  const size_t n_tr = tracing ? c.trace_floats() * (9 + e->D + e->A + kEvalTraceFlags + c.trace_extra) : 1;
  const size_t o_out = carve.add((size_t)N * 4 * 8), o_tr = carve.add(n_tr * 4), o_st = carve.add((size_t)N * kGoalStateFloats * 4),
               o_obs = carve.add((size_t)cdiv(N, 256) * 256 * Dp * 4), o_mu = carve.add((size_t)cdiv(N, 256) * 256 * Ap * 4);
  if (const int rc = grow_eval_buf(e, carve.total)) return rc;
  a.robot_out = eval_at<double>(e, o_out);
  a.st = eval_at<float>(e, o_st);
  a.obs = eval_at<float>(e, o_obs);
  a.mu = eval_at<float>(e, o_mu);
  a.trace = tracing ? eval_at<float>(e, o_tr) : nullptr;
  a.trace_robots = tracing ? c.trace_robots : 0;
  a.trace_steps = tracing ? c.trace_steps : 0;
  a.p = p;
  a.N = N; a.D = e->D; a.Dp = Dp; a.A = e->A; a.Ap = Ap;
  a.deterministic = c.deterministic != 0;
  a.max_steps = c.max_steps;
  a.lo = (float)e->cfg.action_low; a.hi = (float)e->cfg.action_high;
  const uint64_t key = c.seed ^ kEvalKeyMix;
  a.k0 = (uint32_t)key; a.k1 = (uint32_t)(key >> 32);
  a.log_std = Pp(e, T_LOGSTD);
  if (tracing) HIPC(hipMemsetAsync(a.trace, 0, n_tr * 4, e->stream));
  return MOBROB_OK;
}

template <class Task>
static int eval_run(mobrob_ppo_engine_t* e, const typename Task::Args& args, void (*fin)(typename Task::Args)) {
  const EvalArgs& a = Task::eval(args);
  const int N = a.N;
  const bool persistent = e->fused.enabled && e->fused.H == 64 && env_int("MOBROB_EVAL_PERSISTENT", 1) != 0;
  if (persistent) {
    Eval64Net W{Pp(e, e->tPW[0]), Pp(e, e->tPB[0]), Pp(e, e->tPW[1]), Pp(e, e->tPB[1]), Pp(e, T_AW), Pp(e, T_AB)};
    size_t lds_bytes = eval64_lds_bytes(a.Dp);
    if constexpr (Task::kWide) lds_bytes += Task::tile_lds_bytes(args);
    FUSED_DISPATCH_DP(a.Dp, hipLaunchKernelGGL((k_goal64_tile<DPc, Task>), dim3(cdiv(N, 16)), dim3(64), lds_bytes, e->stream, args, W));
  } else {
    hipLaunchKernelGGL(k_goal_task_init<Task>, dim3(cdiv(N, 256)), dim3(256), 0, e->stream, args);
    for (int t = 0; t < a.max_steps; ++t) {
      for (int s = 0; s < N; s += e->rows_max) {
        const int c = std::min(e->rows_max, N - s);
        forward(e, a.obs + (size_t)s * a.Dp, c, true, a.mu + (size_t)s * a.Ap, false, nullptr);
      }
      hipLaunchKernelGGL(k_goal_task_step<Task>, dim3(cdiv(N, 256)), dim3(256), 256 * 33 * sizeof(float), e->stream, args, t);
      if constexpr (task_teams<Task>)
        hipLaunchKernelGGL(k_team_step<typename Task::TeamBase>, dim3(cdiv(N, 256)), dim3(256), 0, e->stream, args, t);
    }
    if (fin) hipLaunchKernelGGL(fin, dim3(cdiv(N, 256)), dim3(256), 0, e->stream, args);
  }
  HIPC(hipGetLastError());
  return persistent ? 1 : 0;
}

static int eval_copy_back(mobrob_ppo_engine_t* e, const EvalCall& c, const EvalArgs& a, double* robot_out, int ran) {
  HIPC(hipMemcpyAsync(robot_out, a.robot_out, (size_t)a.N * 4 * 8, hipMemcpyDeviceToHost, e->stream));
  if (a.trace)
    HIPC(hipMemcpyAsync(c.trace_out, a.trace, c.trace_floats() * (9 + a.D + a.A + kEvalTraceFlags + c.trace_extra) * 4,
                        hipMemcpyDeviceToHost, e->stream));
  HIPC(hipStreamSynchronize(e->stream));
  return ran;
}

struct HazardIO {
  const mobrob_hazards_t* hz;
  double* hazard_out;
  double* episode_cost_out;
  int frames = 0, F = 1, frame_steps = 1, loop = 0;
};
static HazardIO hazard_frames_io(const mobrob_hazard_frames_t* hf, mobrob_hazards_t& view, double* hazard_out, double* episode_cost_out) {
  view = mobrob_hazards_t{hf->n_scenes, hf->max_hazards, hf->hazards, hf->n_hazards, hf->scene, hf->cost, hf->indicator};
  return HazardIO{&view, hazard_out, episode_cost_out, 1, hf->n_frames, hf->frame_steps, hf->loop != 0};
}
struct HazardCarve {
  size_t hz, nhz, scene, out, acc;
  std::vector<int32_t> counts;
};
static int hazard_check(const HazardIO& hio, int N, const char* who, std::vector<int32_t>& counts) {
  const mobrob_hazards_t* hz = hio.hz;
  const int S = hz->n_scenes, M = hz->max_hazards, F = hio.F;
  if (S < 1) return fail(MOBROB_ERR_INVALID, "%s: hazards: n_scenes must be >= 1", who);
  if (M < 0 || M > kHazardMax) return fail(MOBROB_ERR_INVALID, "%s: hazards: max_hazards must lie in 0 .. %d", who, kHazardMax);
  if (hio.frames) {
    if (F < 1) return fail(MOBROB_ERR_INVALID, "%s: hazard frames: n_frames must be >= 1", who);
    if (hio.frame_steps < 1) return fail(MOBROB_ERR_INVALID, "%s: hazard frames: frame_steps must be >= 1", who);
// ... 399 lines not shown
    case MOBROB_BUF_SDE_NOISE:
      if (!e->sde) return fail(MOBROB_ERR_STATE, "the engine was not created with use_sde");
      p = e->sde_E; b = N * (size_t)e->HL * e->A * 4; break;
    default: return fail(MOBROB_ERR_INVALID, "unknown buffer id %d", which);
  }
  if (ptr) *ptr = p;
  if (bytes) *bytes = b;
  return MOBROB_OK;
}

int mobrob_ppo_buffer_info(mobrob_ppo_engine_t* e, int32_t which, void** ptr, size_t* bytes) {
  CHK(buffer_lookup(e, which, ptr, bytes));
  if (ptr && feeds_train_records(which)) e->train_rec_external = true;
  return MOBROB_OK;
}

int mobrob_ppo_read_buffer(mobrob_ppo_engine_t* e, int32_t which, void* host, size_t bytes) {
  if (!e || !host) return fail(MOBROB_ERR_INVALID, "read_buffer: null argument");
  void* p; size_t b;
  CHK(buffer_lookup(e, which, &p, &b));
  if (which == MOBROB_BUF_OBS) {
    const size_t rows = (size_t)(e->T + 1) * e->N;
    if (bytes != rows * e->D * 4) return fail(MOBROB_ERR_INVALID, "read_buffer(OBS): expected %zu bytes", rows * e->D * 4);
    HIPC(hipMemcpy2DAsync(host, (size_t)e->D * 4, p, (size_t)e->Dp * 4, (size_t)e->D * 4, rows, hipMemcpyDeviceToHost, e->stream));
  } else {
    if (bytes != b) return fail(MOBROB_ERR_INVALID, "read_buffer(%d): expected %zu bytes, got %zu", which, b, bytes);
    HIPC(hipMemcpyAsync(host, p, b, hipMemcpyDeviceToHost, e->stream));
  }
  HIPC(hipStreamSynchronize(e->stream));
  return MOBROB_OK;
}

int mobrob_ppo_write_buffer(mobrob_ppo_engine_t* e, int32_t which, const void* host, size_t bytes) {
  if (!e || !host) return fail(MOBROB_ERR_INVALID, "write_buffer: null argument");
  void* p; size_t b;
  CHK(buffer_lookup(e, which, &p, &b));
  if (feeds_train_records(which)) e->train_rec_valid = false;
  if (which == MOBROB_BUF_OBS) {
    const size_t rows = (size_t)(e->T + 1) * e->N;
    if (bytes != rows * e->D * 4) return fail(MOBROB_ERR_INVALID, "write_buffer(OBS): expected %zu bytes", rows * e->D * 4);
    HIPC(hipMemcpy2DAsync(p, (size_t)e->Dp * 4, host, (size_t)e->D * 4, (size_t)e->D * 4, rows, hipMemcpyHostToDevice, e->stream));
  } else {
    if (bytes != b) return fail(MOBROB_ERR_INVALID, "write_buffer(%d): expected %zu bytes, got %zu", which, b, bytes);
    HIPC(hipMemcpyAsync(p, host, b, hipMemcpyHostToDevice, e->stream));
    if (which == MOBROB_BUF_PARAMS) repack(e);
  }
  HIPC(hipStreamSynchronize(e->stream));
  return MOBROB_OK;
}

int mobrob_ppo_feistel_permutation(mobrob_ppo_engine_t* e, int64_t n, uint64_t key, int64_t* out) {
  if (!e || !out || n < 1 || n > ((int64_t)1 << 30)) return fail(MOBROB_ERR_INVALID, "feistel_permutation: bad argument");
  int64_t* d = nullptr;
  HIPC(hipMalloc(&d, (size_t)n * 8));
  hipLaunchKernelGGL(k_perm_feistel, dim3(cdiv((int)n, 256)), dim3(256), 0, e->stream, (int)n, 1, (int)n,
                     feistel_half_bits((uint64_t)n), (uint32_t)key, (uint32_t)(key >> 32), (int*)nullptr, d);
  hipError_t r = hipMemcpyAsync(out, d, (size_t)n * 8, hipMemcpyDeviceToHost, e->stream);
  if (r == hipSuccess) r = hipStreamSynchronize(e->stream);
  (void)hipFree(d);
  if (r != hipSuccess) return fail(MOBROB_ERR_HIP, "feistel_permutation: %s", hipGetErrorString(r));
  return MOBROB_OK;
}

int mobrob_ppo_profile_enable(mobrob_ppo_engine_t* e, int32_t on) {
  if (!e) return fail(MOBROB_ERR_INVALID, "null engine");
  HIPC(hipStreamSynchronize(e->stream));
  prof_resolve(e);
  e->prof_on = on != 0;
  e->prof_mask = on == 1 ? ~0u : (uint32_t)on >> 1;
  for (int i = 0; i < MOBROB_K_COUNT; ++i) { e->prof_ms[i] = 0; e->prof_calls[i] = 0; }
  return MOBROB_OK;
}
int mobrob_ppo_profile_read(mobrob_ppo_engine_t* e, double* ms, int64_t* calls) {
  if (!e) return fail(MOBROB_ERR_INVALID, "null engine");
  HIPC(hipStreamSynchronize(e->stream));
  prof_resolve(e);
  for (int i = 0; i < MOBROB_K_COUNT; ++i) {
    if (ms) ms[i] = e->prof_ms[i];
    if (calls) calls[i] = e->prof_calls[i];
  }
  return MOBROB_OK;
}

#if defined(MOBROB_STAMPS) || defined(MOBROB_PAIR_STAMPS) || defined(MOBROB_EPOCH_STAMPS)
int mobrob_dbg_read_stamps(mobrob_ppo_engine_t* e, unsigned long long* out32, int reset) {
  HIPC(hipStreamSynchronize(e->stream));
  HIPC(hipMemcpy(out32, e->fused.stamps, 32 * 8, hipMemcpyDeviceToHost));
  if (reset) HIPC(hipMemset(e->fused.stamps, 0, 32 * 8));
  return 0;
}
#endif

}
```

### mobrob_amd/csrc/kernels_fused.h

```cpp
#pragma once
#include "device_utils.h"

namespace mobrob {

constexpr int FH = 256;
constexpr int FR = 64;
constexpr int FLDH = FH + 4;
constexpr int FLDO = 36;
constexpr int FTHREADS = 256;

struct FusedNet {
  const f32x4* W1f;
  const f32x4* W2f;
  const f32x4* W3f;
  const f32x4* W3h;
  const f32x4* W2b;
  const f32x4* W3b;
  const float* b1s; const float* b2s;
  const float* b3;
  int head;
  const unsigned* W1x;
  const unsigned* W2x;
  const unsigned* W2bx;
  const unsigned* W1c;
// ... 647 lines not shown
      X3R32_STEP(P0, Q0)
    }
    {
      const int adv = ks + 2 < NKS ? 1 : 0;
      const f32x4 ua = *reinterpret_cast<const f32x4*>(&lds[ao + 16 + 16 * adv]);
      const f32x4 ub = *reinterpret_cast<const f32x4*>(&lds[ao + 20 + 16 * adv]);
#pragma unroll
      for (int pc = 0; pc < 3; ++pc) { P0.p[pc] = b0[(3 + 3 * adv + pc) * 64]; Q0.p[pc] = b1[(3 + 3 * adv + pc) * 64]; }
      X3R32_STEP(P1, Q1)
    }
    ao += 32;
    b0 += 6 * 64;
    b1 += 6 * 64;
  }
  if (NKS & 1) {
    asm volatile("s_nop 1");
    X3R32_MFMA(U, P0, Q0, 1, 1); X3R32_MFMA(U, P0, Q0, 0, 2); X3R32_MFMA(U, P0, Q0, 2, 0);
    X3R32_MFMA(U, P0, Q0, 0, 1); X3R32_MFMA(U, P0, Q0, 1, 0); X3R32_MFMA(U, P0, Q0, 0, 0);
  }
  asm volatile("s_nop 15\n\ts_nop 7" : "+v"(c0), "+v"(c1));
}
template <int LDA, int NKS>
__device__ __forceinline__ void gemm_x3_r64(int a_off, const u32x4* __restrict__ Bx0, const u32x4* __restrict__ Bx1, f32x16& c00,
                                            f32x16& c01, f32x16& c10, f32x16& c11, int lane) {
  constexpr int kAhead = NKS < MOBROB_X3_AHEAD ? NKS : MOBROB_X3_AHEAD;
  const int r = lane & 31, h = lane >> 5;
  const int ab = 4 * opaque((a_off + r * LDA + 8 * h) >> 2);
  X3Frag P[kAhead + 1], Q[kAhead + 1];
#pragma unroll
  for (int k = 0; k < kAhead; ++k) { P[k] = x3_load_b(Bx0, k, lane); Q[k] = x3_load_b(Bx1, k, lane); }
  X3Frag U = x3_split8(*reinterpret_cast<const f32x4*>(&lds[ab]), *reinterpret_cast<const f32x4*>(&lds[ab + 4]));
  X3Frag V = x3_split8(*reinterpret_cast<const f32x4*>(&lds[ab + 32 * LDA]), *reinterpret_cast<const f32x4*>(&lds[ab + 32 * LDA + 4]));
  f32x4 ua = {0.f, 0.f, 0.f, 0.f}, ub = ua, va = ua, vb = ua;
  if (NKS > 1) {
    ua = *reinterpret_cast<const f32x4*>(&lds[ab + 16]);
    ub = *reinterpret_cast<const f32x4*>(&lds[ab + 20]);
    va = *reinterpret_cast<const f32x4*>(&lds[ab + 32 * LDA + 16]);
    vb = *reinterpret_cast<const f32x4*>(&lds[ab + 32 * LDA + 20]);
  }
#pragma unroll
  for (int ks = 0; ks < NKS; ++ks) {
#if MOBROB_X3_PIPE
    __builtin_amdgcn_sched_barrier(0);
#endif
    f32x4 na = ua, nb = ub, ma = va, mb = vb;
    if (ks + 2 < NKS) {
      na = *reinterpret_cast<const f32x4*>(&lds[ab + 16 * (ks + 2)]);
      nb = *reinterpret_cast<const f32x4*>(&lds[ab + 16 * (ks + 2) + 4]);
      ma = *reinterpret_cast<const f32x4*>(&lds[ab + 32 * LDA + 16 * (ks + 2)]);
      mb = *reinterpret_cast<const f32x4*>(&lds[ab + 32 * LDA + 16 * (ks + 2) + 4]);
    }
    if (ks + kAhead < NKS) {
      P[(ks + kAhead) % (kAhead + 1)] = x3_load_b(Bx0, ks + kAhead, lane);
      Q[(ks + kAhead) % (kAhead + 1)] = x3_load_b(Bx1, ks + kAhead, lane);
    }
    const X3Frag& p = P[ks % (kAhead + 1)];
    const X3Frag& q = Q[ks % (kAhead + 1)];
    X3_MFMA6(U, p, c00)
    X3_MFMA6(V, p, c01)
    X3_MFMA6(U, q, c10)
    X3_MFMA6(V, q, c11)
    if (ks + 1 < NKS) { U = x3_split8(ua, ub); V = x3_split8(va, vb); }
    ua = na; ub = nb; va = ma; vb = mb;
#if MOBROB_X3_PIPE
    __builtin_amdgcn_sched_group_barrier(0x100, 4, 0);
    __builtin_amdgcn_sched_group_barrier(0x020, 6, 0);
#pragma unroll
    for (int g = 0; g < 24; ++g) {
      __builtin_amdgcn_sched_group_barrier(0x008, 1, 0);
      __builtin_amdgcn_sched_group_barrier(0x002, 4, 0);
    }
#endif
  }
}
struct PackX3Args {
  const float* W[6]; int N[6], K[6], ld[6], NB[6], KS[6], trans[6];
  float scale[6];
  unsigned short* out[6];
};
__global__ __launch_bounds__(256) void k_pack_x3_multi(PackX3Args a) {
  const int m = blockIdx.y;
  const int i = blockIdx.x * blockDim.x + threadIdx.x;
  const int KS = a.KS[m];
  if (i >= a.NB[m] * KS * 512) return;
  const int j = i & 7, lane = (i >> 3) & 63, ks = (i >> 9) % KS, cb = (i >> 9) / KS;
  const int n = cb * 32 + (lane & 31), k = ks * 16 + 8 * (lane >> 5) + j;
  float x = 0.f;
  if (n < a.N[m] && k < a.K[m]) x = a.scale[m] * (a.trans[m] ? a.W[m][(size_t)k * a.ld[m] + n] : a.W[m][(size_t)n * a.ld[m] + k]);
  asm volatile("" : "+v"(x));
  unsigned p1, p2, p3;
  x3_split2(x, 0.f, p1, p2, p3);
  unsigned short* out = a.out[m];
  const size_t base = ((size_t)(cb * KS + ks) * 3) * 512 + (size_t)lane * 8 + j;
  out[base] = (unsigned short)(p1 & 0xffffu);
  out[base + 512] = (unsigned short)(p2 & 0xffffu);
  out[base + 1024] = (unsigned short)(p3 & 0xffffu);
}

template <int DP>
__device__ __forceinline__ Frag2 tile_layers_x3(const FusedNet& W, int wave, int lane) {
  using L = Lay<DP>;
  const int r_ = lane & 31;
  const u32x4* W1x = reinterpret_cast<const u32x4*>(W.W1x);
  const u32x4* W2x = reinterpret_cast<const u32x4*>(W.W2x);
  {
    const float bz0 = W.b1s[64 * wave + r_], bz1 = W.b1s[64 * wave + 32 + r_];
    f32x16 c00 = splat16(bz0), c01 = splat16(bz0), c10 = splat16(bz1), c11 = splat16(bz1);
    gemm_x3_r64<L::LDX, DP / 16>(L::X, W1x + (size_t)(2 * wave) * (DP / 16) * 192, W1x + (size_t)(2 * wave + 1) * (DP / 16) * 192,
                                 c00, c01, c10, c11, lane);
    store_tanh(L::H1, wave, lane, c00, c01, c10, c11);
  }
  __syncthreads();
  const f32x4* bp = W.W3h;
  Frag2 f3;
  {
    const float bz0 = W.b2s[64 * wave + r_], bz1 = W.b2s[64 * wave + 32 + r_];
    f32x16 c00 = splat16(bz0), c01 = splat16(bz0), c10 = splat16(bz1), c11 = splat16(bz1);
    gemm_x3_r64<FLDH, FH / 16>(L::H1, W2x + (size_t)(2 * wave) * (FH / 16) * 192, W2x + (size_t)(2 * wave + 1) * (FH / 16) * 192,
                               c00, c01, c10, c11, lane);
    f3 = prefetch_frag(bp, bp + 64, lane);
    store_tanh(L::H2, wave, lane, c00, c01, c10, c11);
  }
  __syncthreads();
  return f3;
}

__device__ __forceinline__ void store_tanh_r32(int dst_off, int rb, int wave, int lane, const f32x16& c0, const f32x16& c1) {
  const int r = lane & 31, h = lane >> 5;
  const int o = opaque(dst_off + (32 * rb + 4 * h) * FLDH + 64 * wave + r);
#pragma unroll
  for (int i = 0; i < 16; ++i) {
    lds[o + crc(i) * FLDH] = fast_tanh_scaled(c0[i]);
    lds[o + crc(i) * FLDH + 32] = fast_tanh_scaled(c1[i]);
  }
}
__device__ __forceinline__ void dtanh_inplace_r32(int hs_off, int rb, int wave, int lane, const f32x16& c0, const f32x16& c1) {
  const int r = lane & 31, h = lane >> 5;
  const int o = opaque(hs_off + (32 * rb + 4 * h) * FLDH + 64 * wave + r);
#pragma unroll
  for (int i = 0; i < 16; ++i) {
    float hv;
    hv = lds[o + crc(i) * FLDH];      lds[o + crc(i) * FLDH] = c0[i] * (1.0f - hv * hv);
    hv = lds[o + crc(i) * FLDH + 32]; lds[o + crc(i) * FLDH + 32] = c1[i] * (1.0f - hv * hv);
  }
}
template <int DP, bool H16>
__device__ __forceinline__ Frag2 tile_layers_x3_train(const FusedNet& W, int wave, int lane) {
  using L = Lay<DP>;
  const int r_ = lane & 31;
  const u32x4* W1x = reinterpret_cast<const u32x4*>(W.W1x);
  const u32x4* W2x = reinterpret_cast<const u32x4*>(W.W2x);
  {
    const float bz0 = W.b1s[64 * wave + r_], bz1 = W.b1s[64 * wave + 32 + r_];
#pragma unroll
    for (int rb = 0; rb < 2; ++rb) {
      f32x16 c0 = splat16(bz0), c1 = splat16(bz1);
      gemm_x3_r32_lean<L::LDX, DP / 16>(L::X + rb * 32 * L::LDX, W1x + (size_t)(2 * wave) * (DP / 16) * 192,
                                        W1x + (size_t)(2 * wave + 1) * (DP / 16) * 192, c0, c1, lane);
      store_tanh_r32(L::H1, rb, wave, lane, c0, c1);
    }
  }
  __syncthreads();
  const f32x4* bp = H16 ? W.W3h : W.W3f + (size_t)((wave >> 1) * 16) * 64;
  Frag2 f3;
  {
    const float bz0 = W.b2s[64 * wave + r_], bz1 = W.b2s[64 * wave + 32 + r_];
#pragma unroll
// ... 632 lines not shown
  int nrec = 0;
  unsigned long long todo = __ballot(t >= 0);
  while (todo != 0ull) {
    const int first = __ffsll((long long)todo) - 1;
    const int tsel = __shfl(t, first, 64);
    const bool m = t == tsel;
    const double sum = wave_sum_d(m ? sq : 0.0);
    if (lane == 0 && nrec < kNormRec) { sc[wave * kNormRec + nrec] = sum; sct[wave * kNormRec + nrec] = tsel; }
    ++nrec;
    todo &= ~__ballot(m);
  }
  if (lane == 0)
    for (int k = nrec; k < kNormRec; ++k) sct[wave * kNormRec + k] = -1;
  __syncthreads();
  if (threadIdx.x == 0) {
    int n = 0, cur = -1;
    double acc = 0.0;
    for (int k = 0; k < 4 * kNormRec; ++k) {
      const int tt = sct[k];
      if (tt < 0) continue;
      if (tt == cur) { acc += sc[k]; continue; }
      if (cur >= 0 && n < kNormRec) { stc<COH>(rec_sum + n, acc); stc<COH>(rec_t + n, cur); ++n; }
      cur = tt;
      acc = sc[k];
    }
    if (cur >= 0 && n < kNormRec) { stc<COH>(rec_sum + n, acc); stc<COH>(rec_t + n, cur); ++n; }
    for (; n < kNormRec; ++n) stc<COH>(rec_t + n, -1);
  }
}

__host__ __device__ __forceinline__ int slab_to_canonical(const SlabReduceArgs& s, int net, int p) {
  const int T_W1 = net == 0 ? 1 : 5, T_B1 = net == 0 ? 2 : 6, T_W2 = net == 0 ? 3 : 7, T_B2 = net == 0 ? 4 : 8;
  const int T_W3 = net == 0 ? 9 : 11, T_B3 = net == 0 ? 10 : 12;
  const int head = net == 0 ? s.A : 1;
  auto frag = [](int q, int nt, int* w, int* t, int* i, int* lane) {
    *lane = (q >> 2) & 63;
    *i = (q & 3) + 4 * ((q >> 8) & 3);
    const int wt = q >> 10;
    *t = wt % nt;
    *w = wt / nt;
  };
  int w, t, i, lane;
  if (p < slab_off_w1()) {
    frag(p, 16, &w, &t, &i, &lane);
    const int n = 64 * w + 32 * (t >> 3) + crc(i) + 4 * (lane >> 5), j = 32 * (t & 7) + (lane & 31);
    return s.offs[T_W2] + n * FH + j;
  }
  if (p < slab_off_w3(s.Dp)) {
    frag(p - slab_off_w1(), 4, &w, &t, &i, &lane);
    const int n = 64 * w + 32 * (t >> 1) + crc(i) + 4 * (lane >> 5), j = 32 * (t & 1) + (lane & 31);
    return j < s.D ? s.offs[T_W1] + n * s.D + j : -1;
  }
  if (p < slab_off_b2(s.Dp) && s.h16) {
    const int q = p - slab_off_w3(s.Dp);
    if (q >= 16 * FH) return -1;
    const int e = q & 3, l = (q >> 2) & 63, b = (q >> 8) & 3, w_ = q >> 10;
    const int a_ = 4 * (l >> 4) + e, j = 64 * w_ + 16 * b + (l & 15);
    return a_ < head ? s.offs[T_W3] + a_ * FH + j : -1;
  }
  if (p < slab_off_b2(s.Dp)) {
    frag(p - slab_off_w3(s.Dp), 2, &w, &t, &i, &lane);
    const int a_ = crc(i) + 4 * (lane >> 5), j = 64 * w + 32 * t + (lane & 31);
    return a_ < head ? s.offs[T_W3] + a_ * FH + j : -1;
  }
  if (p < slab_off_b1(s.Dp)) return s.offs[T_B2] + (p - slab_off_b2(s.Dp));
  if (p < slab_off_b3(s.Dp)) return s.offs[T_B1] + (p - slab_off_b1(s.Dp));
  if (p < slab_off_ls(s.Dp)) {
    const int k = p - slab_off_b3(s.Dp);
    return k < head ? s.offs[T_B3] + k : -1;
  }
  if (p < slab_off_st(s.Dp)) {
    const int k = p - slab_off_ls(s.Dp);
    return (net == 0 && k < s.A) ? s.offs[0] + k : -1;
  }
  const int k = p - slab_off_st(s.Dp);
  const bool mine = net == 0 ? (k == 0 || k == 2 || k == 3) : k == 1;
  return mine ? s.P + k : -1;
}

#ifndef MOBROB_SLAB_REDUCE_UNROLL
#define MOBROB_SLAB_REDUCE_UNROLL 8
#endif
constexpr int kSlabReduceUnroll = MOBROB_SLAB_REDUCE_UNROLL;
__global__ __launch_bounds__(256) void k_slab_reduce(SlabReduceArgs s) {
  const int p = blockIdx.x * blockDim.x + threadIdx.x;
  const int net = blockIdx.y;
  if (p == 0 && net == 0) s.sums[4] = s.b_local;
  const int dst = p < s.slab_floats ? slab_to_canonical(s, net, p) : -1;
  float acc = 0.f;
  if (dst >= 0) {
    const float* src = s.slabs + (size_t)net * s.slab_floats + p;
    const size_t stride = 2 * (size_t)s.slab_floats;
    const int n = (s.nslabs - net + 1) / 2;
    constexpr int U = kSlabReduceUnroll;
    float ac[U];
#pragma unroll
    for (int k = 0; k < U; ++k) ac[k] = 0.f;
    int w = 0;
    for (; w + U <= n; w += U) {
      float v[U];
#pragma unroll
      for (int k = 0; k < U; ++k) v[k] = src[(size_t)(w + k) * stride];
#pragma unroll
      for (int k = 0; k < U; ++k) ac[k] += v[k];
    }
#pragma unroll
    for (int k = 0; k < U; ++k)
      if (w + k < n) ac[k] += src[(size_t)(w + k) * stride];
#pragma unroll
    for (int d = U / 2; d >= 1; d >>= 1)
#pragma unroll
      for (int k = 0; k < d; ++k) ac[k] += ac[k + d];
    acc = ac[0];
    if (dst < s.offs[1]) acc = __fadd_rn(acc, __fmul_rn(__fmul_rn(s.ent_coef, -s.b_local), s.inv_bg));
    s.grads[dst] = acc;
  }
  if (s.rec_sum != nullptr) {
    const size_t b = ((size_t)net * gridDim.x + blockIdx.x) * kNormRec;
    block_norm_records(tensor_of_canonical(s.offs, s.P, dst), acc, s.rec_sum + b, s.rec_t + b);
  }
}

__global__ void k_pack_fwd(const float* __restrict__ W, int N, int K, int ld, float* __restrict__ out, int NB,
                           int KG, float scale) {
  const int i = blockIdx.x * blockDim.x + threadIdx.x;
  if (i >= NB * KG * 256) return;
  const int s = i & 3, lane = (i >> 2) & 63, kg = (i >> 8) % KG, nb = (i >> 8) / KG;
  const int n = nb * 32 + (lane & 31), k = kg * 8 + 4 * (lane >> 5) + s;
  out[i] = (n < N && k < K) ? scale * W[(size_t)n * ld + k] : 0.f;
}
__host__ __device__ inline int pack_h16_idx(int n, int k) { return (((k >> 4) * 64) + 16 * ((k >> 2) & 3) + n) * 4 + (k & 3); }
__global__ void k_pack_h16(const float* __restrict__ W, int N, int K, float* __restrict__ out) {
  const int i = blockIdx.x * blockDim.x + threadIdx.x;
  if (i >= (K / 16) * 256) return;
  const int s = i & 3, lane = (i >> 2) & 63, kg = i >> 8;
  const int n = lane & 15, k = 16 * kg + 4 * (lane >> 4) + s;
  out[i] = n < N ? W[(size_t)n * K + k] : 0.f;
}
__global__ void k_scale_copy(const float* __restrict__ src, float* __restrict__ dst, int n, float scale) {
  const int i = blockIdx.x * blockDim.x + threadIdx.x;
  if (i < n) dst[i] = scale * src[i];
}
__global__ void k_pack_bwd(const float* __restrict__ W, int N, int K, int ld, float* __restrict__ out, int JB,
                           int KG) {
  const int i = blockIdx.x * blockDim.x + threadIdx.x;
  if (i >= JB * KG * 256) return;
  const int s = i & 3, lane = (i >> 2) & 63, kg = (i >> 8) % KG, jb = (i >> 8) / KG;
  const int k = kg * 8 + 4 * (lane >> 5) + s, j = jb * 32 + (lane & 31);
  out[i] = (k < N && j < K) ? W[(size_t)k * ld + j] : 0.f;
}

struct FusedActArgs {
  FusedNet net[2];
  const float* X; int Dp; int rows;
  int row0;
  int want_pi, want_v;
  float* mu; int ldmu;
  float* v;
  int sample; int A;
  const float* log_std; const float* eps; uint64_t seed; uint32_t draw; const uint32_t* draw_base; float lo, hi;
  float* act_raw; float* act_clip; float* logp;
};

#define MFMA_KG1(u, p, q)                            \
  _Pragma("unroll") for (int s_ = 0; s_ < 4; ++s_) { \
    c0 = MFMA32(u[s_], p[s_], c0);                   \
    c1 = MFMA32(u[s_], q[s_], c1);                   \
  }
template <int LDA>
__device__ __forceinline__ void gemm_lds_packed_r32(int a_off, const f32x4* __restrict__ Bp0,
                                                    const f32x4* __restrict__ Bp1, int nkg, f32x16& c0, f32x16& c1,
                                                    int lane) {
  const int r = lane & 31, h = lane >> 5;
  const int ab = 4 * opaque((a_off + r * LDA + 4 * h) >> 2);
  unsigned bo = opaque_u((unsigned)lane * 16u);
  f32x4 pA = ldg16(Bp0, bo), qA = ldg16(Bp1, bo), pB, qB;
  f32x4 uA = *reinterpret_cast<const f32x4*>(&lds[ab]), uB;
  int ao = ab;
#pragma unroll 1
  for (int kg = 0; kg < nkg - 2; kg += 2) {
    pB = ldg16(Bp0, bo + 1024u);
// ... 236 lines not shown
  int HL, GL;
  int D, Dp, A, Ap, H1, H2, G1, G2;
  float* pW1p; float* vW1p; float* aWp; float* vWp;
  float* fW1f[2]; float* fW2f[2]; float* fW3f[2]; float* fW3h[2]; float* fW2b[2]; float* fW3b[2]; float* fb1s[2]; float* fb2s[2];
  unsigned short* xW1[2]; unsigned short* xW2[2]; unsigned short* xW2b[2];
  unsigned short* cW1[2]; unsigned short* cW2[2]; unsigned short* cW2b[2]; float* cW3[2]; float* cW3b[2];
  float* stats_row;
  float* loss_sums_zero;
  StatsArgs st;
};

__device__ __forceinline__ int pack_fwd_idx(int n, int k, int KG) {
  return (((n >> 5) * KG + (k >> 3)) * 64 + (n & 31) + 32 * ((k >> 2) & 1)) * 4 + (k & 3);
}
__device__ __forceinline__ int pack_bwd_idx(int krow, int j, int KG) {
  return (((j >> 5) * KG + (krow >> 3)) * 64 + (j & 31) + 32 * ((krow >> 2) & 1)) * 4 + (krow & 3);
}

__device__ __forceinline__ void x3_pack_store(unsigned short* out, int n, int k, int KS, float x) {
  asm volatile("" : "+v"(x));
  unsigned p1, p2, p3;
  x3_split2(x, 0.f, p1, p2, p3);
  const size_t base = ((size_t)((n >> 5) * KS + (k >> 4)) * 3) * 512 + (size_t)((n & 31) + 32 * ((k & 15) >> 3)) * 8 + (k & 7);
  out[base] = (unsigned short)(p1 & 0xffffu);
  out[base + 512] = (unsigned short)(p2 & 0xffffu);
  out[base + 1024] = (unsigned short)(p3 & 0xffffu);
}
__host__ __device__ __forceinline__ void chain_kslot_of_neuron(int n, int* s, int* g, int* j) {
  *s = n >> 5;
  const int r = n & 31;
  *g = (r >> 2) & 3;
  *j = ((r >> 4) << 2) | (r & 3);
}
__host__ __device__ __forceinline__ size_t chain_pack_idx(int unit, int row, int g, int j) {
  return ((size_t)unit * 3) * 512 + (size_t)((row & 15) + 16 * g) * 8 + j;
}
__host__ __device__ __forceinline__ int chain_unit_w1(int tile, int s, int K1) { return tile * K1 + s; }
__host__ __device__ __forceinline__ int chain_unit_w2(int tile, int s) { return s * 16 + tile; }
__host__ __device__ __forceinline__ int chain_unit_w2b(int tile, int s) { return (tile >> 3) * 64 + s * 8 + (tile & 7); }
__device__ __forceinline__ void chain_pack_store(unsigned short* out, size_t base, float x) {
  asm volatile("" : "+v"(x));
  unsigned p1, p2, p3;
  x3_split2(x, 0.f, p1, p2, p3);
  out[base] = (unsigned short)(p1 & 0xffffu);
  out[base + 512] = (unsigned short)(p2 & 0xffffu);
  out[base + 1024] = (unsigned short)(p3 & 0xffffu);
}
__device__ __forceinline__ void chain_store_w1(unsigned short* w1c, int n, int k, int K1, float scaled) {
  chain_pack_store(w1c, chain_pack_idx(chain_unit_w1(n >> 4, k >> 5, K1), n, (k >> 3) & 3, k & 7), scaled);
}
__device__ __forceinline__ void chain_store_w2(unsigned short* w2c, unsigned short* w2bc, int n, int k, float scaled, float raw) {
  int s, g, j;
  chain_kslot_of_neuron(k, &s, &g, &j);
  chain_pack_store(w2c, chain_pack_idx(chain_unit_w2(n >> 4, s), n, g, j), scaled);
  chain_kslot_of_neuron(n, &s, &g, &j);
  chain_pack_store(w2bc, chain_pack_idx(chain_unit_w2b(k >> 4, s), k, g, j), raw);
}
__host__ __device__ __forceinline__ int chain_head_fwd_idx(int a_, int k) { return ((k >> 4) * 64 + a_ + 16 * ((k >> 2) & 3)) * 4 + (k & 3); }
__host__ __device__ __forceinline__ int chain_head_bwd_idx(int a_, int k) { return ((k >> 4) * 64 + (k & 15) + 16 * (a_ >> 2)) * 4 + (a_ & 3); }

template <bool COH = false, class TA = AdamPackArgs>
__device__ __forceinline__ void adam_pack_apply(const TA& a, int i, float graw, float m0, float v0, float p0, float coef, float step_size, float bc2_sqrt) {
  const float g = __fmul_rn(graw, coef);
  const float m = __fmaf_rn(g, 1.0f - a.beta1, __fmul_rn(m0, a.beta1));
  const float v = __fmaf_rn(__fmul_rn(g, g), 1.0f - a.beta2, __fmul_rn(v0, a.beta2));
  const float denom = __fadd_rn(__fdiv_rn(__fsqrt_rn(v), bc2_sqrt), a.eps);
  const float pn = __fmaf_rn(-step_size, __fdiv_rn(m, denom), p0);
  int t = 0;
#pragma unroll
  for (int k = 1; k < kFusedTensors; ++k) t += (i >= a.offs[k]) ? 1 : 0;
  if (a.ntens > kFusedTensors)
    for (int k = kFusedTensors; k < a.ntens; ++k) t += (i >= a.offs[k]) ? 1 : 0;
  const int e = i - a.offs[t];
  a.m[i] = m;
  a.v[i] = v;
  if (COH && a.two_by_two && (t == 0 || t == 10 || t == 12)) stc<true>(a.p + i, pn);
  else a.p[i] = pn;
#ifdef ADAM_NO_PACK
  return;
#endif
  if (!a.two_by_two) {
    if (t == a.id_pw1 || t == a.id_vw1) {
      const int n = e / a.D, k = e - n * a.D;
      (t == a.id_vw1 ? a.vW1p : a.pW1p)[n * a.Dp + k] = pn;
    } else if (t == a.id_aw || t == a.id_vw) {
      (t == a.id_vw ? a.vWp : a.aWp)[e] = pn;
    }
    return;
  }
  switch (t) {
    case 1: case 5: {
      const int net = t == 5, n = e / a.D, k = e - n * a.D;
      (net ? a.vW1p : a.pW1p)[n * a.Dp + k] = pn;
      if (a.fW1f[net]) stc<COH>(a.fW1f[net] + pack_fwd_idx(n, k, a.Dp / 8), kTanhScale * pn);
      if (a.xW1[net]) x3_pack_store(a.xW1[net], n, k, a.Dp / 16, kTanhScale * pn);
      if (a.cW1[net]) chain_store_w1(a.cW1[net], n, k, (a.Dp + 31) / 32, kTanhScale * pn);
    } break;
    case 3: case 7: {
      const int net = t == 7;
      if (a.fW2f[net]) {
        const int K = net ? a.G1 : a.H1, n = e / K, k = e - n * K;
        stc<COH>(a.fW2f[net] + pack_fwd_idx(n, k, K / 8), kTanhScale * pn);
        if (a.fW2b[net]) stc<COH>(a.fW2b[net] + pack_bwd_idx(n, k, (net ? a.G2 : a.H2) / 8), pn);
        if (a.xW2[net]) x3_pack_store(a.xW2[net], n, k, K / 16, kTanhScale * pn);
        if (a.xW2b[net]) x3_pack_store(a.xW2b[net], k, n, (net ? a.G2 : a.H2) / 16, pn);
        if (a.cW2[net]) chain_store_w2(a.cW2[net], a.cW2b[net], n, k, kTanhScale * pn, pn);
      }
    } break;
    case 9: case 11: {
      const int net = t == 11, K = net ? a.G2 : a.H2, n = e / K, k = e - n * K;
      (net ? a.vWp : a.aWp)[e] = pn;
      if (a.fW3f[net]) {
        stc<COH>(a.fW3f[net] + pack_fwd_idx(n, k, K / 8), pn);
        if (a.fW3b[net]) stc<COH>(a.fW3b[net] + pack_bwd_idx(n, k, 4), pn);
        if (a.fW3h[net] && n < 16) stc<COH>(a.fW3h[net] + pack_h16_idx(n, k), pn);
        if (a.cW3[net] && n < 16) { a.cW3[net][chain_head_fwd_idx(n, k)] = pn; a.cW3b[net][chain_head_bwd_idx(n, k)] = pn; }
      }
    } break;
    case 2: case 6: if (a.fb1s[t == 6]) stc<COH>(a.fb1s[t == 6] + e, kTanhScale * pn); break;
    case 4: case 8: if (a.fb2s[t == 8]) stc<COH>(a.fb2s[t == 8] + e, kTanhScale * pn); break;
    default: break;
  }
}

template <bool COH, class TA>
__device__ __forceinline__ void adam_pack_block_at(const TA& a, int lin, int i, float g_in, float m_in, float v_in, float p_in, float step_size,
                                                   float bc2_sqrt, float* stats_row, float inv_bg, float ent_pre, int fidx_pre = -1) {
  __shared__ double part[1024];
  __shared__ int tens[256];
  __shared__ float nts[kMaxTensors + 3];
  __shared__ float coef_s, total_s;
  if (lin == 0 && a.st.loss_sums != nullptr) {
    StatsArgs st;
    st.stats_row = stats_row; st.loss_sums = a.st.loss_sums; st.log_std = a.st.log_std;
    st.ent_coef = a.st.ent_coef; st.vf_coef = a.st.vf_coef; st.inv_bg = inv_bg; st.n_act = a.st.n_act; st.sde = a.st.sde;
    stats_row_from_sums<COH>(st, ent_pre);
  }
  if (a.fold_idx != nullptr) {
    const int nrec = a.fold_start[13];
    if (nrec <= 128) {
      if ((int)threadIdx.x < nrec) part[threadIdx.x] = ldc<COH>(a.partial + (fidx_pre >= 0 ? fidx_pre : a.fold_idx[threadIdx.x]));
      __syncthreads();
      if (threadIdx.x < 13) {
        double ts = 0.0;
        for (int c = a.fold_start[threadIdx.x]; c < a.fold_start[threadIdx.x + 1]; ++c) ts += part[c];
        nts[threadIdx.x] = (float)sqrt(ts);
      }
    } else {
      const int lane = threadIdx.x & 63, wv = threadIdx.x >> 6;
      const bool staged = nrec <= 1024;
      if (staged) {
        for (int c = threadIdx.x; c < nrec; c += blockDim.x) part[c] = ldc<COH>(a.partial + a.fold_idx[c]);
        __syncthreads();
      }
      for (int t = wv; t < 13; t += 4) {
        double ts = 0.0;
        if (staged)
          for (int c = a.fold_start[t] + lane; c < a.fold_start[t + 1]; c += 64) ts += part[c];
        else
          for (int c = a.fold_start[t] + lane; c < a.fold_start[t + 1]; c += 64) ts += ldc<COH>(a.partial + a.fold_idx[c]);
        ts = wave_sum_d(ts);
        if (lane == 0) nts[t] = (float)sqrt(ts);
      }
    }
  } else {
    for (int c = threadIdx.x; c < a.nchunks; c += blockDim.x) {
      part[c] = ldc<COH>(a.partial + c);
      tens[c] = a.chunks[c].tensor;
    }
    __syncthreads();
    if ((int)threadIdx.x < a.ntens) {
      double ts = 0.0;
      for (int c = 0; c < a.nchunks; ++c)
        if (tens[c] == (int)threadIdx.x) ts += part[c];
      nts[threadIdx.x] = (float)sqrt(ts);
    }
  }
  __syncthreads();
  if (threadIdx.x == 0) {
    float tot_sq = 0.f;
    for (int t = 0; t < a.ntens; ++t) tot_sq = __fmaf_rn(nts[t], nts[t], tot_sq);
    const float total = sqrtf(tot_sq);
    total_s = total;
    coef_s = fminf(a.max_norm / (total + 1e-6f), 1.0f);
  }
  __syncthreads();
  const float coef = coef_s;
  if (lin == 0 && stats_row != nullptr) stats_row[6] = total_s;
  if (lin < 8 && a.loss_sums_zero != nullptr) stc<COH>(a.loss_sums_zero + lin, 0.f);
  if (i < 0 || i >= a.P) return;
  adam_pack_apply<COH>(a, i, g_in, m_in, v_in, p_in, coef, step_size, bc2_sqrt);
}
template <bool COH, class TA>
__device__ __forceinline__ void adam_pack_block(const TA& a, int bx, float step_size, float bc2_sqrt, float* stats_row, float inv_bg) {
  const int i = bx * 256 + (int)threadIdx.x;
  float g_in = 0.f, m_in = 0.f, v_in = 0.f, p_in = 0.f;
  if (i < a.P) { g_in = ldc<COH>(a.g + i); m_in = ldc<COH>(a.m + i); v_in = ldc<COH>(a.v + i); p_in = ldc<COH>(a.p + i); }
  const float ent = (i == 0 && a.st.loss_sums != nullptr) ? entropy_of_log_std<COH>(a.st.log_std, a.st.n_act) : 0.f;
  adam_pack_block_at<COH>(a, i, i, g_in, m_in, v_in, p_in, step_size, bc2_sqrt, stats_row, inv_bg, ent);
}
__global__ __launch_bounds__(256) void k_adam_pack(AdamPackArgs a) {
  adam_pack_block<false>(a, blockIdx.x, a.step_size, a.bc2_sqrt, a.stats_row, a.st.inv_bg);
}

struct FusedState {
  bool enabled = false;
  int H = 0;
  int D = 0, Dp = 0, A = 0;
  float* packed = nullptr;
  size_t packed_floats = 0;
  FusedNet net[2];
  float* slabs = nullptr;
  float* train_rec = nullptr;
  bool train_x3 = false;
  bool train_chain = false;
  size_t lds_chain_bytes = 0;
  unsigned long long* stamps = nullptr;
  int slab_floats = 0, max_grid = 0;
  int pair_nseq_max = 0;
  size_t lds_bytes = 0, lds_act_bytes = 0;
};

inline size_t fused_lds_bytes(int Dp) { return (size_t)(FR * (Dp + 4) + 2 * FR * FLDH + FR * FLDO + 96 + 256 + 16) * sizeof(float); }

inline size_t fused_lds_act_bytes(int Dp) { return (size_t)(32 * (Dp + 4) + 2 * 32 * FLDH + 4 * 32 * FLDO) * sizeof(float); }

inline int padded_obs_dim(int D) { return D <= 64 ? (D + 15) / 16 * 16 : (D + 7) / 8 * 8; }
inline bool fused_shape_ok(int D, int A, int H1, int H2, int G1, int G2) {
  const int Dp = padded_obs_dim(D);
  const bool same = H1 == H2 && H1 == G1 && H1 == G2 && (H1 == FH || H1 == 64);
  return same && A <= 32 && (Dp == 16 || Dp == 32 || Dp == 48 || Dp == 64);
}

inline void fused_repack(FusedState& f, const float* params, const int* offs, hipStream_t st) {
  if (!f.enabled) return;
  const int Dp = f.Dp, D = f.D, A = f.A;
  auto fwd = [&](const float* W, int N, int K, int ld, const f32x4* out, int NB, int KG, float scale) {
    hipLaunchKernelGGL(k_pack_fwd, dim3((NB * KG * 256 + 255) / 256), dim3(256), 0, st, W, N, K, ld, (float*)out, NB, KG,
                       scale);
  };
  auto bwd = [&](const float* W, int N, int K, int ld, const f32x4* out, int JB, int KG) {
    hipLaunchKernelGGL(k_pack_bwd, dim3((JB * KG * 256 + 255) / 256), dim3(256), 0, st, W, N, K, ld, (float*)out, JB, KG);
  };
  const int w1[2] = {1, 5}, w2[2] = {3, 7}, w3[2] = {9, 11}, heads[2] = {A, 1};
  const int H = f.H;
  for (int n = 0; n < 2; ++n) {
    fwd(params + offs[w1[n]], H, D, D, f.net[n].W1f, H / 32, Dp / 8, kTanhScale);
    fwd(params + offs[w2[n]], H, H, H, f.net[n].W2f, H / 32, H / 8, kTanhScale);
    fwd(params + offs[w3[n]], heads[n], H, H, f.net[n].W3f, 1, H / 8, 1.0f);
    if (heads[n] <= 16)
      hipLaunchKernelGGL(k_pack_h16, dim3(H / 16), dim3(256), 0, st, params + offs[w3[n]], heads[n], H, (float*)f.net[n].W3h);
    hipLaunchKernelGGL(k_scale_copy, dim3(1), dim3(256), 0, st, params + offs[w1[n] + 1], (float*)f.net[n].b1s, H, kTanhScale);
    hipLaunchKernelGGL(k_scale_copy, dim3(1), dim3(256), 0, st, params + offs[w2[n] + 1], (float*)f.net[n].b2s, H, kTanhScale);
    bwd(params + offs[w2[n]], H, H, H, f.net[n].W2b, H / 32, H / 8);
    bwd(params + offs[w3[n]], heads[n], H, H, f.net[n].W3b, H / 32, 4);
  }
}

inline void fused_launch_act(FusedState& f, FusedActArgs& a, hipStream_t st);

inline bool fused_forward(FusedState& f, const float* X, int rows, bool want_pi, float* mu_out, int ldmu, bool want_v,
                          float* v_out, hipStream_t st) {
  if (!f.enabled) return false;
  FusedActArgs a{};
  a.X = X; a.rows = rows; a.want_pi = want_pi; a.want_v = want_v; a.mu = mu_out; a.ldmu = ldmu; a.v = v_out;
  a.sample = 0; a.A = f.A;
  fused_launch_act(f, a, st);
  return true;
}

}
```

Baseline: 31.99 million.

## Defer rollout-only weight packing out of per-minibatch Adam into lazy repack

During an update, the Adam pack kernel no longer writes the padded and forward-packed weight copies that only rollout and inference use. Instead it marks them stale, and they are rebuilt once by launching the pack kernels before the next rollout, act, predict or eval call. This removes scattered stores from every optimizer step in exchange for a single repack per update. The diff also adds an optional multi-load grouping in slab reduce (off by default) and a debug read entry point.

```diff
diff --git a/mobrob_amd/csrc/engine.hip b/mobrob_amd/csrc/engine.hip
--- a/mobrob_amd/csrc/engine.hip
+++ b/mobrob_amd/csrc/engine.hip
@@ -194,6 +194,8 @@
   double* norm_rec_sum = nullptr; int* norm_rec_t = nullptr; int* fold_idx_dev = nullptr;
   int fold_start[kMaxTensors + 1] = {0};
   bool use_norm_records = false;
+  bool lean_adam = false;
+  bool rollout_packs_stale = false;
   bool epoch_kernel_on = true;
   unsigned* epoch_bar = nullptr;
   float* epoch_consts = nullptr;
@@ -429,7 +431,7 @@
 float* Pp(mobrob_ppo_engine* e, int t) { return e->params + e->offs[t]; }
 float* Gp(mobrob_ppo_engine* e, int t) { return e->grads + e->offs[t]; }
 
-void pack_x3_all(mobrob_ppo_engine* e) {
+void pack_x3_all(mobrob_ppo_engine* e, bool forward_only = false) {
   if (e->fused.net[0].W2x == nullptr) return;
   PackX3Args a{};
   const int w1[2] = {T_PW1, T_VW1}, w2[2] = {T_PW2, T_VW2};
@@ -441,11 +443,11 @@
     a.W[i2] = Pp(e, w2[n]); a.N[i2] = FH; a.K[i2] = FH; a.ld[i2] = FH; a.NB[i2] = FH / 32; a.KS[i2] = FH / 16; a.scale[i2] = kTanhScale;
     a.out[i2] = reinterpret_cast<unsigned short*>(const_cast<unsigned*>(e->fused.net[n].W2x));
     a.W[i3] = Pp(e, w2[n]); a.N[i3] = FH; a.K[i3] = FH; a.ld[i3] = FH; a.NB[i3] = FH / 32; a.KS[i3] = FH / 16; a.scale[i3] = 1.0f; a.trans[i3] = 1;
-    a.out[i3] = reinterpret_cast<unsigned short*>(const_cast<unsigned*>(e->fused.net[n].W2bx));
+    a.out[i3] = forward_only ? nullptr : reinterpret_cast<unsigned short*>(const_cast<unsigned*>(e->fused.net[n].W2bx));
     maxthreads = std::max(maxthreads, std::max(a.NB[i1] * a.KS[i1], a.NB[i2] * a.KS[i2]) * 512);
   }
   hipLaunchKernelGGL(k_pack_x3_multi, dim3(cdiv(maxthreads, 256), 6), dim3(256), 0, e->stream, a);
-  if (e->fused.train_chain) {
+  if (e->fused.train_chain && !forward_only) {
     ChainPackArgs c{};
     const int w3[2] = {T_AW, T_VW};
     for (int n = 0; n < 2; ++n) {
@@ -461,7 +463,7 @@
   }
 }
 
-void repack(mobrob_ppo_engine* e) {
+void repack_padded(mobrob_ppo_engine* e) {
   auto pad = [&](const float* src, float* dst, int r, int c, int rp, int cp) {
     hipLaunchKernelGGL(k_pad_rows, dim3(cdiv(rp * cp, 256)), dim3(256), 0, e->stream, src, dst, r, c, rp, cp);
   };
@@ -469,8 +471,19 @@
   pad(Pp(e, T_VW1), e->vW1p, e->G1, e->D, e->G1, e->Dp);
   pad(Pp(e, T_AW), e->aWp, e->A, e->HL, e->Ap, e->HL);
   pad(Pp(e, T_VW), e->vWp, 1, e->GL, 8, e->GL);
+}
+void repack(mobrob_ppo_engine* e) {
+  repack_padded(e);
   fused_repack(e->fused, e->params, e->offs, e->stream);
   pack_x3_all(e);
+  e->rollout_packs_stale = false;
+}
+void ensure_rollout_packs(mobrob_ppo_engine* e) {
+  if (!e->rollout_packs_stale) return;
+  repack_padded(e);
+  fused_repack(e->fused, e->params, e->offs, e->stream, true);
+  pack_x3_all(e, true);
+  e->rollout_packs_stale = false;
 }
 
 void forward_generic(mobrob_ppo_engine* e, const float* X, int rows, bool want_pi, float* mu_out, bool want_v,
@@ -1285,6 +1298,7 @@
 
 int mobrob_ppo_rollout_begin(mobrob_ppo_engine_t* e) {
   if (!e) return fail(MOBROB_ERR_INVALID, "null engine");
+  ensure_rollout_packs(e);
   e->t = 0;
   e->rollout_ready = false; e->train_rec_valid = false;
   e->nparts = 0;
@@ -1301,6 +1315,7 @@
 int mobrob_ppo_act(mobrob_ppo_engine_t* e, const float* obs, const float* eps, float* a_raw, float* a_clip,
                    float* values, float* logp) {
   if (!e || !obs) return fail(MOBROB_ERR_INVALID, "act: null argument");
+  ensure_rollout_packs(e);
   if (e->t >= e->T) return fail(MOBROB_ERR_STATE, "act: rollout buffer full (t=%d, n_steps=%d)", e->t, e->T);
   CHK(streamer_init(e));
   const size_t N = e->N, A = e->A, D = e->D;
@@ -1369,6 +1384,7 @@
 int mobrob_ppo_store(mobrob_ppo_engine_t* e, const float* rewards, const uint8_t* dones, const uint8_t* truncated,
                      const float* terminal_obs) {
   if (!e || !rewards || !dones) return fail(MOBROB_ERR_INVALID, "store: null argument");
+  ensure_rollout_packs(e);
   if (e->t >= e->T) return fail(MOBROB_ERR_STATE, "store: rollout buffer full");
   CHK(streamer_init(e));
   const size_t N = e->N, D = e->D;
@@ -1421,6 +1437,7 @@
 
 int mobrob_ppo_act_part(mobrob_ppo_engine_t* e, int32_t part, int32_t nparts, const float* obs, float* a_clip) {
   if (!e || !obs || !a_clip) return fail(MOBROB_ERR_INVALID, "act_part: null argument");
+  ensure_rollout_packs(e);
   int r0, n;
   CHK(part_range(e, part, nparts, &r0, &n));
   const int t = e->part_act_t[part];
@@ -1452,6 +1469,7 @@
                           const uint8_t* dones, const uint8_t* truncated, const float* terminal_obs,
                           const float* next_obs) {
   if (!e || !rewards || !dones) return fail(MOBROB_ERR_INVALID, "store_part: null argument");
+  ensure_rollout_packs(e);
   int r0, n;
   CHK(part_range(e, part, nparts, &r0, &n));
   const int t = e->part_store_t[part];
@@ -1484,6 +1502,7 @@
 
 int mobrob_ppo_finish_rollout(mobrob_ppo_engine_t* e, const float* last_obs, const uint8_t* dones) {
   if (!e || !last_obs || !dones) return fail(MOBROB_ERR_INVALID, "finish_rollout: null argument");
+  ensure_rollout_packs(e);
   if (e->t != e->T) return fail(MOBROB_ERR_STATE, "finish_rollout: %d of %d steps stored", e->t, e->T);
   CHK(streamer_init(e));
   const size_t N = e->N;
@@ -1718,6 +1737,7 @@
 }
 
 int collect_device(mobrob_ppo_engine* e, const mobrob_ppo_engine::RolloutSpec& sp) {
+  ensure_rollout_packs(e);
   const int N = e->N, Dp = e->Dp, per = Dp / 4;
   const size_t slot = (size_t)N * Dp;
   if (e->env_started != sp.kind) {
@@ -2215,6 +2235,7 @@
   if (!e) return fail(MOBROB_ERR_INVALID, "null engine");
   if (!e->epoch_open) return fail(MOBROB_ERR_STATE, "minibatch_grad before epoch_begin");
   if (mb < 0 || mb >= e->nmb) return fail(MOBROB_ERR_INVALID, "minibatch %d out of range [0,%d)", mb, e->nmb);
+  if (!e->lean_adam) ensure_rollout_packs(e);
   const int start = mb * e->Bl, B = std::min(e->Bl, e->N * e->T - start);
   const float inv_bg = 1.0f / (float)((int64_t)B * e->cfg.world_size);
   e->cur_count = B;
@@ -2239,21 +2260,22 @@
   for (int i = 0; i <= kMaxTensors; ++i) a.offs[i] = e->offs[i];
   a.ntens = e->ntens; a.two_by_two = e->Lp == 2 && e->Lv == 2; a.id_pw1 = T_PW1; a.id_vw1 = T_VW1; a.id_aw = T_AW; a.id_vw = T_VW; a.HL = e->HL; a.GL = e->GL;
   a.D = e->D; a.Dp = e->Dp; a.A = e->A; a.Ap = e->Ap; a.H1 = e->H1; a.H2 = e->H2; a.G1 = e->G1; a.G2 = e->G2;
-  a.pW1p = e->pW1p; a.vW1p = e->vW1p; a.aWp = e->aWp; a.vWp = e->vWp;
+  const bool lean = e->lean_adam;
+  if (!lean) { a.pW1p = e->pW1p; a.vW1p = e->vW1p; a.aWp = e->aWp; a.vWp = e->vWp; }
   for (int n = 0; n < 2; ++n) {
     const bool on = e->fused.enabled;
-    a.fW1f[n] = on ? (float*)e->fused.net[n].W1f : nullptr;
-    a.fW2f[n] = on ? (float*)e->fused.net[n].W2f : nullptr;
-    a.fW3f[n] = on ? (float*)e->fused.net[n].W3f : nullptr;
+    a.fW1f[n] = on && !lean ? (float*)e->fused.net[n].W1f : nullptr;
+    a.fW2f[n] = on && !lean ? (float*)e->fused.net[n].W2f : nullptr;
+    a.fW3f[n] = on && !lean ? (float*)e->fused.net[n].W3f : nullptr;
     const bool ch = on && e->fused.train_chain;
     a.fW2b[n] = on && !ch ? (float*)e->fused.net[n].W2b : nullptr;
     a.fW3b[n] = on && !ch ? (float*)e->fused.net[n].W3b : nullptr;
-    a.fW3h[n] = (on && (n == 1 || e->fused.A <= 16)) ? (float*)e->fused.net[n].W3h : nullptr;
+    a.fW3h[n] = (on && !lean && (n == 1 || e->fused.A <= 16)) ? (float*)e->fused.net[n].W3h : nullptr;
     a.fb1s[n] = on ? (float*)e->fused.net[n].b1s : nullptr;
     a.fb2s[n] = on ? (float*)e->fused.net[n].b2s : nullptr;
     const bool x3 = on && e->fused.train_x3;
-    a.xW1[n] = x3 ? reinterpret_cast<unsigned short*>(const_cast<unsigned*>(e->fused.net[n].W1x)) : nullptr;
-    a.xW2[n] = x3 ? reinterpret_cast<unsigned short*>(const_cast<unsigned*>(e->fused.net[n].W2x)) : nullptr;
+    a.xW1[n] = x3 && !lean ? reinterpret_cast<unsigned short*>(const_cast<unsigned*>(e->fused.net[n].W1x)) : nullptr;
+    a.xW2[n] = x3 && !lean ? reinterpret_cast<unsigned short*>(const_cast<unsigned*>(e->fused.net[n].W2x)) : nullptr;
     a.xW2b[n] = x3 && !ch ? reinterpret_cast<unsigned short*>(const_cast<unsigned*>(e->fused.net[n].W2bx)) : nullptr;
     a.cW1[n] = ch ? reinterpret_cast<unsigned short*>(const_cast<unsigned*>(e->fused.net[n].W1c)) : nullptr;
     a.cW2[n] = ch ? reinterpret_cast<unsigned short*>(const_cast<unsigned*>(e->fused.net[n].W2c)) : nullptr;
@@ -2293,6 +2315,7 @@
   a.stats_row = st.stats_row;
   a.loss_sums_zero = e->fused.enabled ? e->grads + e->P : nullptr;
   hipLaunchKernelGGL(k_adam_pack, dim3(cdiv(e->P, 256)), dim3(256), 0, e->stream, a);
+  if (e->lean_adam) e->rollout_packs_stale = true;
   HIPC(hipGetLastError());
   e->grad_pending = false;
   return MOBROB_OK;
@@ -2494,6 +2517,9 @@
 }
 
 namespace {
+bool lean_adam_wanted(bool fused_on, int H, bool train_chain) {
+  return fused_on && H == FH && train_chain && !env_switched_off("MOBROB_NO_LEAN_ADAM");
+}
 bool norm_records_wanted(const mobrob_ppo_engine* e, bool dp) {
   return !dp && e->fused.enabled && e->target_kl <= 0.0 && !env_switched_off("MOBROB_NO_NORM_RECORDS");
 }
@@ -2578,6 +2604,11 @@
     RecordsOn(mobrob_ppo_engine* e_, bool on) : e(e_) { e->use_norm_records = on; }
     ~RecordsOn() { e->use_norm_records = false; }
   } records_on(e, records);
+  struct LeanOn {
+    mobrob_ppo_engine* e;
+    explicit LeanOn(mobrob_ppo_engine* e_) : e(e_) { e->lean_adam = lean_adam_wanted(e->fused.enabled, e->fused.H, e->fused.train_chain); }
+    ~LeanOn() { e->lean_adam = false; ensure_rollout_packs(e); }
+  } lean_on(e);
   EpochLaunch epoch_launch;
   const bool epoch_kernel = epoch_kernel_eligible(e, dp, records, &epoch_launch);
   e->last_update_mode = epoch_kernel ? 1 : 0;
@@ -2871,6 +2902,7 @@
 int mobrob_ppo_predict(mobrob_ppo_engine_t* e, const float* obs, int32_t n, int32_t deterministic, const float* eps,
                        float* actions, float* values) {
   if (!e || !obs || n < 1) return fail(MOBROB_ERR_INVALID, "predict: bad argument");
+  ensure_rollout_packs(e);
   for (int s = 0; s < n; s += e->rows_max) {
     const int c = std::min(e->rows_max, n - s);
     CHK(upload_obs(e, obs + (size_t)s * e->D, e->pred_obs, c));
@@ -2970,6 +3002,7 @@
 static T* eval_at(const mobrob_ppo_engine_t* e, size_t off) { return reinterpret_cast<T*>(e->eval_buf + off); }
 
 static int eval_prepare(mobrob_ppo_engine_t* e, const EvalCall& c, const GoalEnvParams& p, EvalCarve& carve, EvalArgs& a) {
+  ensure_rollout_packs(e);
   const int N = c.N, Dp = e->Dp, Ap = e->Ap;
   const bool tracing = c.tracing();
   const size_t n_tr = tracing ? c.trace_floats() * (9 + e->D + e->A + kEvalTraceFlags + c.trace_extra) : 1;
@@ -3535,6 +3568,63 @@
   return MOBROB_OK;
 }
 
+int mobrob_dbg_read(mobrob_ppo_engine_t* e, int32_t what, void* out, size_t cap, size_t* bytes) {
+  if (!e || !bytes) return fail(MOBROB_ERR_INVALID, "dbg_read: null argument");
+  const FusedState& f = e->fused;
+  std::vector<std::pair<const void*, size_t>> parts;
+  std::vector<int32_t> host;
+  const bool wide = f.enabled && f.H == FH;
+  const size_t nx1 = wide ? (size_t)(FH / 32) * (e->Dp / 16) * 192 * 16 : 0, nx2 = (size_t)(FH / 32) * (FH / 16) * 192 * 16;
+  const int nb = f.enabled ? cdiv(f.slab_floats, 256) : 0;
+  switch (what) {
+    case 0:
+      parts = {{e->pW1p, (size_t)e->H1 * e->Dp * 4}, {e->vW1p, (size_t)e->G1 * e->Dp * 4}, {e->aWp, (size_t)e->Ap * e->HL * 4}, {e->vWp, (size_t)8 * e->GL * 4}};
+      break;
+    case 1: if (f.enabled) parts = {{f.packed, f.packed_floats * 4}}; break;
+    case 2: if (wide && f.net[0].W2x) for (int n = 0; n < 2; ++n) { parts.push_back({f.net[n].W1x, nx1}); parts.push_back({f.net[n].W2x, nx2}); } break;
+    case 3: if (wide && f.net[0].W2x) for (int n = 0; n < 2; ++n) parts.push_back({f.net[n].W2bx, nx2}); break;
+    case 4:
+      if (wide && f.train_chain)
+        for (int n = 0; n < 2; ++n) {
+          parts.push_back({f.net[n].W1c, (size_t)((e->Dp + 31) / 32) * 16 * 768 * 4}); parts.push_back({f.net[n].W2c, (size_t)8 * 16 * 768 * 4});
+          parts.push_back({f.net[n].W2bc, (size_t)8 * 16 * 768 * 4}); parts.push_back({f.net[n].W3c, (size_t)16 * 64 * 4 * 4});
+          parts.push_back({f.net[n].W3bc, (size_t)16 * 64 * 4 * 4});
+        }
+      break;
+    case 5: if (wide) parts = {{f.slabs, (size_t)f.max_grid * f.slab_floats * 4}}; break;
+    case 6: if (f.enabled) parts = {{e->norm_rec_sum, (size_t)2 * nb * kNormRec * 8}}; break;
+    case 7: if (f.enabled) parts = {{e->norm_rec_t, (size_t)2 * nb * kNormRec * 4}}; break;
+    case 8: {
+      if (!f.enabled) break;
+      for (int t = 0; t <= 13; ++t) host.push_back(e->fold_start[t]);
+      std::vector<int32_t> idx((size_t)e->fold_start[13]);
+      HIPC(hipStreamSynchronize(e->stream));
+      if (!idx.empty()) HIPC(hipMemcpy(idx.data(), e->fold_idx_dev, idx.size() * 4, hipMemcpyDeviceToHost));
+      host.insert(host.end(), idx.begin(), idx.end());
+    } break;
+    case 9: host = {e->rollout_packs_stale ? 1 : 0, e->lean_adam ? 1 : 0}; break;
+    default: return fail(MOBROB_ERR_INVALID, "dbg_read: what = %d", what);
+  }
+  if (!host.empty()) {
+    *bytes = host.size() * 4;
+    if (out) memcpy(out, host.data(), std::min(cap, *bytes));
+    return MOBROB_OK;
+  }
+  size_t total = 0;
+  for (auto& q : parts) total += q.second;
+  *bytes = total;
+  if (!out) return MOBROB_OK;
+  HIPC(hipStreamSynchronize(e->stream));
+  size_t done = 0;
+  for (auto& q : parts) {
+    if (done >= cap) break;
+    const size_t n = std::min(q.second, cap - done);
+    HIPC(hipMemcpy((char*)out + done, q.first, n, hipMemcpyDeviceToHost));
+    done += n;
+  }
+  return MOBROB_OK;
+}
+
 #if defined(MOBROB_STAMPS) || defined(MOBROB_PAIR_STAMPS) || defined(MOBROB_EPOCH_STAMPS)
 int mobrob_dbg_read_stamps(mobrob_ppo_engine_t* e, unsigned long long* out32, int reset) {
   HIPC(hipStreamSynchronize(e->stream));
diff --git a/mobrob_amd/csrc/kernels_fused.h b/mobrob_amd/csrc/kernels_fused.h
--- a/mobrob_amd/csrc/kernels_fused.h
+++ b/mobrob_amd/csrc/kernels_fused.h
@@ -753,7 +753,7 @@
   const int m = blockIdx.y;
   const int i = blockIdx.x * blockDim.x + threadIdx.x;
   const int KS = a.KS[m];
-  if (i >= a.NB[m] * KS * 512) return;
+  if (a.out[m] == nullptr || i >= a.NB[m] * KS * 512) return;
   const int j = i & 7, lane = (i >> 3) & 63, ks = (i >> 9) % KS, cb = (i >> 9) / KS;
   const int n = cb * 32 + (lane & 31), k = ks * 16 + 8 * (lane >> 5) + j;
   float x = 0.f;
@@ -1552,6 +1552,11 @@
 #define MOBROB_SLAB_REDUCE_UNROLL 8
 #endif
 constexpr int kSlabReduceUnroll = MOBROB_SLAB_REDUCE_UNROLL;
+#ifndef MOBROB_SLAB_REDUCE_LOADS
+#define MOBROB_SLAB_REDUCE_LOADS MOBROB_SLAB_REDUCE_UNROLL
+#endif
+constexpr int kSlabReduceLoads = MOBROB_SLAB_REDUCE_LOADS;
+static_assert(kSlabReduceLoads % kSlabReduceUnroll == 0, "the load group is a whole number of accumulator rounds");
 __global__ __launch_bounds__(256) void k_slab_reduce(SlabReduceArgs s) {
   const int p = blockIdx.x * blockDim.x + threadIdx.x;
   const int net = blockIdx.y;
@@ -1567,6 +1572,16 @@
 #pragma unroll
     for (int k = 0; k < U; ++k) ac[k] = 0.f;
     int w = 0;
+    if constexpr (kSlabReduceLoads > U) {
+      constexpr int L = kSlabReduceLoads;
+      for (; w + L <= n; w += L) {
+        float v[L];
+#pragma unroll
+        for (int k = 0; k < L; ++k) v[k] = src[(size_t)(w + k) * stride];
+#pragma unroll
+        for (int k = 0; k < L; ++k) ac[k % U] += v[k];
+      }
+    }
     for (; w + U <= n; w += U) {
       float v[U];
 #pragma unroll
@@ -1969,25 +1984,28 @@
   if (!a.two_by_two) {
     if (t == a.id_pw1 || t == a.id_vw1) {
       const int n = e / a.D, k = e - n * a.D;
-      (t == a.id_vw1 ? a.vW1p : a.pW1p)[n * a.Dp + k] = pn;
+      float* w1p = t == a.id_vw1 ? a.vW1p : a.pW1p;
+      if (w1p) w1p[n * a.Dp + k] = pn;
     } else if (t == a.id_aw || t == a.id_vw) {
-      (t == a.id_vw ? a.vWp : a.aWp)[e] = pn;
+      float* wp = t == a.id_vw ? a.vWp : a.aWp;
+      if (wp) wp[e] = pn;
     }
     return;
   }
   switch (t) {
     case 1: case 5: {
       const int net = t == 5, n = e / a.D, k = e - n * a.D;
-      (net ? a.vW1p : a.pW1p)[n * a.Dp + k] = pn;
+      float* w1p = net ? a.vW1p : a.pW1p;
+      if (w1p) w1p[n * a.Dp + k] = pn;
       if (a.fW1f[net]) stc<COH>(a.fW1f[net] + pack_fwd_idx(n, k, a.Dp / 8), kTanhScale * pn);
       if (a.xW1[net]) x3_pack_store(a.xW1[net], n, k, a.Dp / 16, kTanhScale * pn);
       if (a.cW1[net]) chain_store_w1(a.cW1[net], n, k, (a.Dp + 31) / 32, kTanhScale * pn);
     } break;
     case 3: case 7: {
       const int net = t == 7;
-      if (a.fW2f[net]) {
+      if (a.fW2f[net] || a.cW2[net]) {
         const int K = net ? a.G1 : a.H1, n = e / K, k = e - n * K;
-        stc<COH>(a.fW2f[net] + pack_fwd_idx(n, k, K / 8), kTanhScale * pn);
+        if (a.fW2f[net]) stc<COH>(a.fW2f[net] + pack_fwd_idx(n, k, K / 8), kTanhScale * pn);
         if (a.fW2b[net]) stc<COH>(a.fW2b[net] + pack_bwd_idx(n, k, (net ? a.G2 : a.H2) / 8), pn);
         if (a.xW2[net]) x3_pack_store(a.xW2[net], n, k, K / 16, kTanhScale * pn);
         if (a.xW2b[net]) x3_pack_store(a.xW2b[net], k, n, (net ? a.G2 : a.H2) / 16, pn);
@@ -1996,9 +2014,10 @@
     } break;
     case 9: case 11: {
       const int net = t == 11, K = net ? a.G2 : a.H2, n = e / K, k = e - n * K;
-      (net ? a.vWp : a.aWp)[e] = pn;
-      if (a.fW3f[net]) {
-        stc<COH>(a.fW3f[net] + pack_fwd_idx(n, k, K / 8), pn);
+      float* wp = net ? a.vWp : a.aWp;
+      if (wp) wp[e] = pn;
+      if (a.fW3f[net] || a.cW3[net]) {
+        if (a.fW3f[net]) stc<COH>(a.fW3f[net] + pack_fwd_idx(n, k, K / 8), pn);
         if (a.fW3b[net]) stc<COH>(a.fW3b[net] + pack_bwd_idx(n, k, 4), pn);
         if (a.fW3h[net] && n < 16) stc<COH>(a.fW3h[net] + pack_h16_idx(n, k), pn);
         if (a.cW3[net] && n < 16) { a.cW3[net][chain_head_fwd_idx(n, k)] = pn; a.cW3b[net][chain_head_bwd_idx(n, k)] = pn; }
@@ -2119,7 +2138,7 @@
   return same && A <= 32 && (Dp == 16 || Dp == 32 || Dp == 48 || Dp == 64);
 }
 
-inline void fused_repack(FusedState& f, const float* params, const int* offs, hipStream_t st) {
+inline void fused_repack(FusedState& f, const float* params, const int* offs, hipStream_t st, bool forward_only = false) {
   if (!f.enabled) return;
   const int Dp = f.Dp, D = f.D, A = f.A;
   auto fwd = [&](const float* W, int N, int K, int ld, const f32x4* out, int NB, int KG, float scale) {
@@ -2137,6 +2156,7 @@
     fwd(params + offs[w3[n]], heads[n], H, H, f.net[n].W3f, 1, H / 8, 1.0f);
     if (heads[n] <= 16)
       hipLaunchKernelGGL(k_pack_h16, dim3(H / 16), dim3(256), 0, st, params + offs[w3[n]], heads[n], H, (float*)f.net[n].W3h);
+    if (forward_only) continue;
     hipLaunchKernelGGL(k_scale_copy, dim3(1), dim3(256), 0, st, params + offs[w1[n] + 1], (float*)f.net[n].b1s, H, kTanhScale);
     hipLaunchKernelGGL(k_scale_copy, dim3(1), dim3(256), 0, st, params + offs[w2[n] + 1], (float*)f.net[n].b2s, H, kTanhScale);
     bwd(params + offs[w2[n]], H, H, H, f.net[n].W2b, H / 32, H / 8);
```

Result: no change. 31.82 million (-0.5%).
